# Rita-zi/WavTokenizer

Measured on AMD Instinct MI355X. Metric: audio-seconds/sec encode+decode, 24 kHz 3 s clips, higher is better.
Workload: dtype f32 (split-f16 x3 products)

## Files before the change

include/wavtokenizer_amd.h:

```cpp
#ifndef WAVTOKENIZER_AMD_H
#define WAVTOKENIZER_AMD_H

#include <stddef.h>
#include <stdint.h>

#ifdef __cplusplus
extern "C" {
#endif

typedef enum {
    WT_OK = 0,
    WT_ERR_INVALID = -1,
    WT_ERR_MISSING_TENSOR = -2,
    WT_ERR_SHAPE = -3,
    WT_ERR_HIP = -4,
    WT_ERR_NOT_INITED = -5,
    WT_ERR_RANGE = -6,
    WT_ERR_LSTM_SYNC = -7,
    WT_ERR_INDEX = -8
} wt_status;

enum wt_status_bits {
    WT_STATUS_BIT_LSTM = 1,
    WT_STATUS_BIT_RANGE = 2
// ... 37 lines not shown
    WT_PLAN_FLAG_STEP_LSTM = 4,
    WT_PLAN_FLAG_GRAPH = 8,
    WT_PLAN_FLAG_FP32_GEMM = 2,
    WT_PLAN_FLAG_RANGE_REPORT = 32,
    WT_PLAN_FLAG_MIXED_LENGTH = 64
};

enum wt_range_site {
    WT_SITE_ENCODER = 0,
    WT_SITE_BB_EMBED = 1,
    WT_SITE_RES0 = 2, WT_SITE_RES1 = 3,
    WT_SITE_ATTN = 4,
    WT_SITE_RES2 = 5, WT_SITE_RES3 = 6,
    WT_SITE_CNX0 = 7,
    WT_SITE_HEAD = 40,
    WT_SITE_SEANET_DECODER = 41
};

const char* wt_last_error(void);
const char* wt_version(void);

int  wt_model_create(const wt_arch* arch, const wt_tensor* tensors, int32_t n_tensors, int32_t device,
                     wt_model** out);
void wt_model_destroy(wt_model* m);

size_t wt_model_export_bytes(const wt_model* m);
int  wt_model_export(const wt_model* m, void* buf, size_t n);
int  wt_packed_info(const void* buf, size_t n, wt_arch* arch, int32_t* version, uint64_t* arch_hash);
int  wt_packed_verify(const void* buf, size_t n);
size_t wt_packed_bytes(const void* buf, size_t n);
int  wt_model_create_packed(const void* buf, size_t n, int32_t device, wt_model** out);
int  wt_model_hop(const wt_model* m);
int  wt_model_persistent_lstm(const wt_model* m);
int  wt_device_info(int32_t device, int32_t* compute_units, int32_t* is_gfx950, int32_t* persistent_lstm);
int64_t wt_model_weight_bytes(const wt_model* m);

int    wt_plan_create(const wt_model* m, int32_t kind, int32_t B, int64_t len, int32_t flags, wt_plan** out);
int    wt_plan_create_ex(const wt_model* m, int32_t kind, int32_t B, int64_t len, int32_t flags, uint64_t fp32_sites,
                         wt_plan** out);
void   wt_plan_destroy(wt_plan* p);
size_t wt_plan_workspace_bytes(const wt_plan* p);
int64_t wt_plan_frames(const wt_plan* p);
int    wt_plan_num_launches(const wt_plan* p);
int64_t wt_plan_graph_replays(const wt_plan* p);
int    wt_plan_find_buffer(const wt_plan* p, const char* name, size_t* offset, size_t* numel);
int    wt_plan_buffer_info(const wt_plan* p, const char* name, size_t* offset, size_t* numel, int32_t* format);
int    wt_plan_status(const wt_plan* p, int32_t* bits, int32_t clear);
int    wt_plan_range_sites(const wt_plan* p, uint64_t* sites, int32_t clear);
int    wt_plan_range_report(const wt_plan* p, int32_t index, const char** step, const char** buffer, float* amax);
int    wt_model_status(const wt_model* m, int32_t* bits, int32_t clear);
int    wt_model_split_ok(const wt_model* m);
int    wt_plan_buffer_name(const wt_plan* p, int32_t index, const char** name);

int wt_plan_num_steps(const wt_plan* p);
int wt_plan_step_name(const wt_plan* p, int32_t index, const char** name);
int wt_plan_set_timing(const wt_plan* p, const char* name_substr);
int wt_plan_read_timing(const wt_plan* p, double* total_ms, int64_t* launches, int32_t reset);

int wt_encode(const wt_plan* p, const float* wav, float* features, int64_t* codes, float* emb_out,
              void* workspace, void* stream);

int wt_encode_mixed(const wt_plan* p, const float* wav, const int32_t* lengths, float* features, int64_t* codes, float* emb_out,
                    void* workspace, void* stream);
int64_t wt_plan_min_clip_length(const wt_plan* p);
int wt_sconv_geometry(int64_t T, int32_t k, int32_t stride, int32_t dilation, int32_t out[4]);

int wt_codes_to_features(const wt_model* m, const int64_t* codes, int32_t K, int32_t B, int64_t L,
                         float* features, void* stream);

int wt_decode(const wt_plan* p, const float* features, int32_t bandwidth_id, float* wav_out,
              float* backbone_out, void* workspace, void* stream);

int wt_head(const wt_plan* p, const float* x, float* wav_out, void* workspace, void* stream);

int wt_seanet_decode(const wt_plan* p, const float* features, float* wav_out, void* workspace, void* stream);


int wt_sconv1d(const float* x, const float* w, const float* bias, float* y, int32_t B, int64_t T,
               int32_t Cin, int32_t Cout, int32_t k, int32_t stride, int32_t dilation, int32_t elu_input,
               void* stream);

int wt_linear(const float* x, const float* w, const float* bias, float* y, int64_t M, int32_t N, int32_t K,
              int32_t f16x3, void* workspace, void* stream);

int wt_conv1d_s32(const float* x, const float* w, const float* bias, float* y, int32_t B, int64_t T, int32_t Cin,
                  int32_t Cout, int32_t k, int32_t stride, int32_t zero_same, void* workspace, void* stream);

size_t wt_vq_workspace_bytes(int64_t N, int32_t D, int32_t bins);
int wt_vq_nearest(const float* x, const float* embed, int64_t N, int32_t D, int32_t bins, int64_t* codes_out,
                  void* workspace, void* stream);
int wt_vq_nearest_f32(const float* x, const float* embed, int64_t N, int32_t D, int32_t bins, int64_t* codes_out,
                      void* workspace, void* stream);

typedef struct {
    int32_t size;
    int32_t engine, epi, out, pro, b_is_act;
    int32_t M, N, K;
    int32_t T_in, T_out, Cin, taps, stride, dil, pad_left, pad_mode, Tp;
    int32_t K1, nz, tap_pair, head_kb;
    float alpha;
    int64_t a_bstride, a_rstride, a2_bstride, a2_rstride, w_rstride, c_rstride, r_rstride, zA, zW, zC;
    const float* A;
    const float* A2;
    const float* B;
    const float* bias;
    const float* R;
    const float* gamma;
    float* C;
    float* C2;
    uint32_t* status;
} wt_gemm_desc;
typedef struct {
    int32_t BM, BN, waves_m, waves_n, stages, ks, prod, staged, bias_cache, G, tiles;
} wt_launch_form;
size_t wt_gemm_probe_workspace_bytes(const wt_gemm_desc* d);
int wt_gemm_probe(const wt_gemm_desc* d, wt_launch_form* form, void* workspace, void* stream);

enum { WT_OP_GN_APPLY = 0, WT_OP_GN_STATS = 1, WT_OP_ROWNORM = 2, WT_OP_SOFTMAX = 3, WT_OP_ISTFT_OLA = 4, WT_OP_CONV_FIRST = 5,
       WT_OP_CONV_LAST = 6, WT_OP_TRANSPOSE = 7, WT_OP_CONVTR = 8, WT_OP_ROW_SUMSQ = 9, WT_OP_S32_AMAX = 10 };
enum { WT_OPK_GN_TILE = 1, WT_OPK_GN_CHUNK = 2, WT_OPK_GN_STATS = 3, WT_OPK_ROWNORM = 4, WT_OPK_DWCONV_LN = 5,
       WT_OPK_SOFTMAX_REG = 6, WT_OPK_SOFTMAX_RMW = 7, WT_OPK_ISTFT_OLA = 8, WT_OPK_CONV_FIRST = 9, WT_OPK_CONV_LAST32 = 10,
       WT_OPK_CONV_LAST = 11, WT_OPK_TRANSPOSE = 12, WT_OPK_CONVTR = 13, WT_OPK_ROW_SUMSQ = 14, WT_OPK_S32_AMAX = 15 };
typedef struct {
    int32_t size;
    int32_t op;
    int32_t B, L, C;
    int32_t groups, mode, flag, out_s32;
    int32_t ld, k, stride, Cout, n_fft, hop, Kq;
    float eps;
    int64_t n;
    const void* x;
    const void *p0, *p1, *p2, *p3, *p4, *p5;
    void *y, *y2, *y3;
    uint32_t* status;
} wt_op_desc;
typedef struct {
    int32_t kernel;
    int32_t variant;
    int32_t variant2;
    int32_t grid_x, grid_y, grid_z, block, lds;
} wt_op_form;
int wt_op_probe(const wt_op_desc* d, wt_op_form* form, void* stream);

int wt_resblock(const float* x, const float* wav, const float* e0_w, const float* e0_b, const float* w3, const float* b3,
                const float* w1, const float* b1, const float* ws, const float* bs, float* y, int32_t B, int64_t T,
                int32_t C, int32_t elu_out, int32_t out_s32, int32_t fp32_chain, void* stream);
int wt_resblock_down(const float* wav, const float* e0_w, const float* e0_b, const float* w3, const float* b3, const float* w1,
                     const float* b1, const float* ws, const float* bs, const float* wd, const float* bd, float* y_down,
                     int32_t B, int64_t T, int32_t r, void* stream);

int wt_unit_run(const wt_plan* p, const float* x, float* y, void* workspace, void* stream);

int wt_model_take_bad_codes(const wt_model* m);


typedef struct wt_resampler wt_resampler;
int     wt_resampler_create(int32_t orig_sr, int32_t new_sr, int32_t device, wt_resampler** out);
void    wt_resampler_destroy(wt_resampler* r);
int64_t wt_resampler_out_length(const wt_resampler* r, int64_t T);
int     wt_convert_audio(const wt_resampler* r, const float* wav, int32_t B, int32_t C, int64_t T, float* out, void* stream);

int wt_pcm16(const float* x, int64_t n, float limit, int32_t rescale, int16_t* out, void* workspace, void* stream);

int wt_linear_overlap_add(const float* frames, const float* weight, int32_t n_frames, int64_t rows, int64_t frame_len,
                          int64_t last_len, int64_t stride, float* out, void* stream);

#ifdef __cplusplus
}
#endif
#endif
```

wavtokenizer_amd/_capi.py:

```python
from __future__ import annotations

import ctypes
import os
from ctypes import POINTER, c_char_p, c_float, c_int32, c_int64, c_size_t, c_void_p

_HERE = os.path.dirname(os.path.abspath(__file__))
LIB_PATH = os.environ.get("WAVTOK_HIP_LIB") or os.path.join(_HERE, "libwavtok_hip.so")

EXPORTS = [
    "wt_last_error", "wt_version", "wt_model_create", "wt_model_destroy", "wt_model_export_bytes", "wt_model_export", "wt_packed_info", "wt_packed_verify", "wt_packed_bytes",
    "wt_model_create_packed", "wt_model_hop", "wt_model_weight_bytes",
    "wt_plan_create", "wt_plan_create_ex", "wt_plan_range_sites", "wt_plan_range_report", "wt_model_persistent_lstm", "wt_device_info", "wt_plan_destroy", "wt_plan_workspace_bytes", "wt_plan_frames", "wt_plan_num_launches", "wt_plan_graph_replays",
    "wt_plan_find_buffer", "wt_plan_buffer_info", "wt_plan_buffer_name", "wt_plan_status", "wt_plan_num_steps", "wt_plan_step_name",
    "wt_plan_set_timing", "wt_plan_read_timing", "wt_model_split_ok", "wt_model_status", "wt_model_take_bad_codes", "wt_encode", "wt_codes_to_features",
    "wt_decode", "wt_seanet_decode", "wt_head", "wt_unit_run", "wt_sconv1d", "wt_linear", "wt_conv1d_s32", "wt_vq_workspace_bytes",
    "wt_vq_nearest", "wt_vq_nearest_f32", "wt_resblock", "wt_resblock_down", "wt_gemm_probe_workspace_bytes", "wt_gemm_probe", "wt_op_probe",
    "wt_resampler_create", "wt_resampler_destroy", "wt_resampler_out_length", "wt_convert_audio", "wt_pcm16",
    "wt_linear_overlap_add", "wt_encode_mixed", "wt_plan_min_clip_length", "wt_sconv_geometry",
]

WT_PLAN_ENCODE, WT_PLAN_DECODE, WT_PLAN_SEANET_DECODER, WT_PLAN_HEAD, WT_PLAN_UNIT_LSTM = 0, 1, 2, 3, 4
WT_PLAN_FLAG_KEEP_STAGES = 1
WT_PLAN_FLAG_FP32_GEMM = 2
WT_PLAN_FLAG_STEP_LSTM = 4
WT_PLAN_FLAG_GRAPH = 8
WT_PLAN_FLAG_UNFUSED = 16
WT_PLAN_FLAG_RANGE_REPORT = 32
WT_PLAN_FLAG_MIXED_LENGTH = 64
WT_SITE_ENCODER, WT_SITE_BB_EMBED, WT_SITE_RES0, WT_SITE_RES1, WT_SITE_ATTN, WT_SITE_RES2, WT_SITE_RES3 = 0, 1, 2, 3, 4, 5, 6
WT_SITE_CNX0, WT_SITE_HEAD, WT_SITE_SEANET_DECODER = 7, 40, 41
WT_ERR_INVALID = -1
WT_ERR_RANGE, WT_ERR_LSTM_SYNC, WT_ERR_INDEX = -6, -7, -8
WT_STATUS_BIT_LSTM, WT_STATUS_BIT_RANGE = 1, 2
BUF_S32, BUF_ELU = 1, 2


class WtArch(ctypes.Structure):
    _fields_ = [("n_ratios", c_int32), ("ratios", c_int32 * 8), ("vq_bins", c_int32), ("num_quantizers", c_int32),
                ("input_channels", c_int32), ("dim", c_int32), ("intermediate_dim", c_int32),
                ("num_layers", c_int32), ("adanorm_num_embeddings", c_int32), ("n_fft", c_int32),
                ("hop_length", c_int32), ("padding_same", c_int32)]


class WtTensor(ctypes.Structure):
    _fields_ = [("name", c_char_p), ("data", POINTER(c_float)), ("numel", c_int64)]


class WtGemmDesc(ctypes.Structure):
    _fields_ = ([("size", c_int32), ("engine", c_int32), ("epi", c_int32), ("out", c_int32), ("pro", c_int32), ("b_is_act", c_int32),
                 ("M", c_int32), ("N", c_int32), ("K", c_int32)]
                + [(n, c_int32) for n in ("T_in", "T_out", "Cin", "taps", "stride", "dil", "pad_left", "pad_mode", "Tp",
                                         "K1", "nz", "tap_pair", "head_kb")]
                + [("alpha", c_float)]
                + [(n, c_int64) for n in ("a_bstride", "a_rstride", "a2_bstride", "a2_rstride", "w_rstride", "c_rstride",
                                         "r_rstride", "zA", "zW", "zC")]
                + [(n, c_void_p) for n in ("A", "A2", "B", "bias", "R", "gamma", "C", "C2", "status")])


class WtLaunchForm(ctypes.Structure):
    _fields_ = [(n, c_int32) for n in ("BM", "BN", "waves_m", "waves_n", "stages", "ks", "prod", "staged", "bias_cache", "G", "tiles")]


WT_OP_GN_APPLY, WT_OP_GN_STATS, WT_OP_ROWNORM, WT_OP_SOFTMAX, WT_OP_ISTFT_OLA, WT_OP_CONV_FIRST = 0, 1, 2, 3, 4, 5
WT_OP_CONV_LAST, WT_OP_TRANSPOSE, WT_OP_CONVTR, WT_OP_ROW_SUMSQ, WT_OP_S32_AMAX = 6, 7, 8, 9, 10
WT_OPK_NAMES = {1: "gn_tile", 2: "gn_chunk", 3: "gn_stats", 4: "rownorm", 5: "dwconv_ln", 6: "softmax_reg", 7: "softmax_rmw",
                8: "istft_ola", 9: "conv_first", 10: "conv_last32", 11: "conv_last", 12: "transpose", 13: "convtr",
                14: "row_sumsq", 15: "s32_amax"}


class WtOpDesc(ctypes.Structure):
    _fields_ = ([(n, c_int32) for n in ("size", "op", "B", "L", "C", "groups", "mode", "flag", "out_s32", "ld", "k", "stride",
                                        "Cout", "n_fft", "hop", "Kq")]
                + [("eps", c_float), ("n", c_int64)]
                + [(n, c_void_p) for n in ("x", "p0", "p1", "p2", "p3", "p4", "p5", "y", "y2", "y3", "status")])


class WtOpForm(ctypes.Structure):
    _fields_ = [(n, c_int32) for n in ("kernel", "variant", "variant2", "grid_x", "grid_y", "grid_z", "block", "lds")]


class WavTokError(RuntimeError):
    def __init__(self, msg, status=0):
        super().__init__(msg)
        self.status = status


def _load() -> ctypes.CDLL:
    if not os.path.exists(LIB_PATH):
        raise ImportError(
            f"{LIB_PATH} not found: build the HIP extension first (python -c 'import __graft_entry__ as g; g.build()' "
            "or make -C wavtokenizer_amd/csrc). There is no CPU fallback for the product path.")
    lib = ctypes.CDLL(LIB_PATH)
    if os.environ.get("WAVTOK_HIP_LIB"):
        class _Missing:
            def __init__(self, name):
                self.name, self.argtypes, self.restype = name, None, None

            def __call__(self, *a):
                raise WavTokError(f"{LIB_PATH} has no {self.name}")
        for sym in EXPORTS:
            try:
                getattr(lib, sym)
            except AttributeError:
                setattr(lib, sym, _Missing(sym))
    lib.wt_last_error.restype = c_char_p
    lib.wt_version.restype = c_char_p
    lib.wt_model_create.argtypes = [POINTER(WtArch), POINTER(WtTensor), c_int32, c_int32, POINTER(c_void_p)]
    lib.wt_model_destroy.argtypes = [c_void_p]
    lib.wt_model_destroy.restype = None
    lib.wt_model_export_bytes.argtypes = [c_void_p]
    lib.wt_model_export_bytes.restype = c_size_t
    lib.wt_model_export.argtypes = [c_void_p, c_void_p, c_size_t]
    lib.wt_packed_info.argtypes = [c_void_p, c_size_t, POINTER(WtArch), POINTER(c_int32), POINTER(ctypes.c_uint64)]
    lib.wt_packed_verify.argtypes = [c_void_p, c_size_t]
    lib.wt_packed_bytes.argtypes = [c_void_p, c_size_t]
    lib.wt_packed_bytes.restype = c_size_t
    lib.wt_model_create_packed.argtypes = [c_void_p, c_size_t, c_int32, POINTER(c_void_p)]
    lib.wt_model_hop.argtypes = [c_void_p]
    lib.wt_model_weight_bytes.argtypes = [c_void_p]
    lib.wt_model_weight_bytes.restype = c_int64
    lib.wt_plan_create.argtypes = [c_void_p, c_int32, c_int32, c_int64, c_int32, POINTER(c_void_p)]
    lib.wt_plan_create_ex.argtypes = [c_void_p, c_int32, c_int32, c_int64, c_int32, ctypes.c_uint64, POINTER(c_void_p)]
    lib.wt_plan_range_sites.argtypes = [c_void_p, POINTER(ctypes.c_uint64), c_int32]
    lib.wt_plan_range_report.argtypes = [c_void_p, c_int32, POINTER(c_char_p), POINTER(c_char_p), POINTER(c_float)]
    lib.wt_model_persistent_lstm.argtypes = [c_void_p]
    lib.wt_device_info.argtypes = [c_int32, POINTER(c_int32), POINTER(c_int32), POINTER(c_int32)]
    lib.wt_plan_destroy.argtypes = [c_void_p]
    lib.wt_plan_destroy.restype = None
    lib.wt_plan_workspace_bytes.argtypes = [c_void_p]
    lib.wt_plan_workspace_bytes.restype = c_size_t
    lib.wt_plan_frames.argtypes = [c_void_p]
    lib.wt_plan_frames.restype = c_int64
    lib.wt_plan_num_launches.argtypes = [c_void_p]
    lib.wt_plan_graph_replays.argtypes = [c_void_p]
    lib.wt_plan_graph_replays.restype = c_int64
    lib.wt_plan_find_buffer.argtypes = [c_void_p, c_char_p, POINTER(c_size_t), POINTER(c_size_t)]
    lib.wt_plan_buffer_info.argtypes = [c_void_p, c_char_p, POINTER(c_size_t), POINTER(c_size_t), POINTER(c_int32)]
    lib.wt_plan_status.argtypes = [c_void_p, POINTER(c_int32), c_int32]
    lib.wt_model_split_ok.argtypes = [c_void_p]
    lib.wt_model_status.argtypes = [c_void_p, POINTER(c_int32), c_int32]
    lib.wt_model_take_bad_codes.argtypes = [c_void_p]
    lib.wt_unit_run.argtypes = [c_void_p, c_void_p, c_void_p, c_void_p, c_void_p]
    lib.wt_plan_buffer_name.argtypes = [c_void_p, c_int32, POINTER(c_char_p)]
    lib.wt_plan_num_steps.argtypes = [c_void_p]
    lib.wt_plan_step_name.argtypes = [c_void_p, c_int32, POINTER(c_char_p)]
    lib.wt_plan_set_timing.argtypes = [c_void_p, c_char_p]
    lib.wt_plan_read_timing.argtypes = [c_void_p, POINTER(ctypes.c_double), POINTER(c_int64), c_int32]
    lib.wt_encode.argtypes = [c_void_p, c_void_p, c_void_p, c_void_p, c_void_p, c_void_p, c_void_p]
    lib.wt_encode_mixed.argtypes = [c_void_p, c_void_p, c_void_p, c_void_p, c_void_p, c_void_p, c_void_p, c_void_p]
    lib.wt_plan_min_clip_length.argtypes = [c_void_p]
    lib.wt_plan_min_clip_length.restype = c_int64
    lib.wt_sconv_geometry.argtypes = [c_int64, c_int32, c_int32, c_int32, POINTER(c_int32)]
    lib.wt_codes_to_features.argtypes = [c_void_p, c_void_p, c_int32, c_int32, c_int64, c_void_p, c_void_p]
    lib.wt_decode.argtypes = [c_void_p, c_void_p, c_int32, c_void_p, c_void_p, c_void_p, c_void_p]
    lib.wt_seanet_decode.argtypes = [c_void_p, c_void_p, c_void_p, c_void_p, c_void_p]
    lib.wt_head.argtypes = [c_void_p, c_void_p, c_void_p, c_void_p, c_void_p]
    lib.wt_sconv1d.argtypes = [c_void_p, c_void_p, c_void_p, c_void_p, c_int32, c_int64, c_int32, c_int32, c_int32,
                               c_int32, c_int32, c_int32, c_void_p]
    lib.wt_linear.argtypes = [c_void_p, c_void_p, c_void_p, c_void_p, c_int64, c_int32, c_int32, c_int32, c_void_p, c_void_p]
    lib.wt_conv1d_s32.argtypes = [c_void_p, c_void_p, c_void_p, c_void_p, c_int32, c_int64, c_int32, c_int32, c_int32,
                                  c_int32, c_int32, c_void_p, c_void_p]
    lib.wt_vq_workspace_bytes.argtypes = [c_int64, c_int32, c_int32]
    lib.wt_vq_workspace_bytes.restype = c_size_t
    lib.wt_vq_nearest.argtypes = [c_void_p, c_void_p, c_int64, c_int32, c_int32, c_void_p, c_void_p, c_void_p]
    lib.wt_vq_nearest_f32.argtypes = [c_void_p, c_void_p, c_int64, c_int32, c_int32, c_void_p, c_void_p, c_void_p]
    lib.wt_resblock.argtypes = [c_void_p] * 11 + [c_int32, c_int64, c_int32, c_int32, c_int32, c_int32, c_void_p]
    lib.wt_resblock_down.argtypes = [c_void_p] * 12 + [c_int32, c_int64, c_int32, c_void_p]
    lib.wt_gemm_probe_workspace_bytes.argtypes = [POINTER(WtGemmDesc)]
    lib.wt_gemm_probe_workspace_bytes.restype = c_size_t
    lib.wt_gemm_probe.argtypes = [POINTER(WtGemmDesc), POINTER(WtLaunchForm), c_void_p, c_void_p]
    lib.wt_op_probe.argtypes = [POINTER(WtOpDesc), POINTER(WtOpForm), c_void_p]
    lib.wt_resampler_create.argtypes = [c_int32, c_int32, c_int32, POINTER(c_void_p)]
    lib.wt_resampler_destroy.argtypes = [c_void_p]
    lib.wt_resampler_destroy.restype = None
    lib.wt_resampler_out_length.argtypes = [c_void_p, c_int64]
    lib.wt_resampler_out_length.restype = c_int64
    lib.wt_convert_audio.argtypes = [c_void_p, c_void_p, c_int32, c_int32, c_int64, c_void_p, c_void_p]
    lib.wt_pcm16.argtypes = [c_void_p, c_int64, ctypes.c_float, c_int32, c_void_p, c_void_p, c_void_p]
    lib.wt_linear_overlap_add.argtypes = [c_void_p, c_void_p, c_int32, c_int64, c_int64, c_int64, c_int64, c_void_p, c_void_p]
    return lib


lib = _load()


def check(rc: int, what: str = "") -> None:
    if rc != 0:
        msg = lib.wt_last_error()
        raise WavTokError(f"{what} failed (status {rc}): {msg.decode() if msg else ''}", rc)
```

wavtokenizer_amd/csrc/capi.cpp:

```cpp
#include "model.h"

namespace wt {
static thread_local std::string g_err;
void set_error(const std::string& msg) { g_err = msg; }
thread_local LaunchCtx g_launch;
int device_cus() {
    static std::atomic<int> cache[64];
    int d = 0;
    (void)hipGetDevice(&d);
    d &= 63;
    int v = cache[d].load(std::memory_order_relaxed);
    if (v <= 0) {
        if (hipDeviceGetAttribute(&v, hipDeviceAttributeMultiprocessorCount, d) != hipSuccess || v <= 0) v = 256;
        cache[d].store(v, std::memory_order_relaxed);
    }
    return v;
}
}

using namespace wt;

static int alloc_host_words(wt_model* M, const char* who) {
    void* hp = nullptr;
    void* dp = nullptr;
// ... 547 lines not shown
    return run_plan(p, c);
}

int wt_decode(const wt_plan* p, const float* features, int32_t bandwidth_id, float* wav_out, float* backbone_out,
              void* workspace, void* stream) {
    if (!p || p->kind != WT_PLAN_DECODE) { set_error("wt_decode: not a decode plan"); return WT_ERR_INVALID; }
    if (!features || !wav_out || !workspace) { set_error("wt_decode: null buffer"); return WT_ERR_INVALID; }
    if (bandwidth_id < 0 || bandwidth_id >= p->model->arch.adanorm_num_embeddings) {
        set_error("wt_decode: bandwidth_id out of range"); return WT_ERR_INVALID;
    }
    RunCtx c{static_cast<char*>(workspace), static_cast<hipStream_t>(stream), features, wav_out, nullptr, backbone_out, bandwidth_id};
    return run_plan(p, c);
}

int wt_head(const wt_plan* p, const float* x, float* wav_out, void* workspace, void* stream) {
    if (!p || p->kind != WT_PLAN_HEAD) { set_error("wt_head: wrong plan kind"); return WT_ERR_INVALID; }
    if (!x || !wav_out || !workspace) { set_error("wt_head: null buffer"); return WT_ERR_INVALID; }
    RunCtx c{static_cast<char*>(workspace), static_cast<hipStream_t>(stream), x, wav_out, nullptr, nullptr, 0};
    return run_plan(p, c);
}

int wt_seanet_decode(const wt_plan* p, const float* features, float* wav_out, void* workspace, void* stream) {
    if (!p || p->kind != WT_PLAN_SEANET_DECODER) { set_error("wt_seanet_decode: wrong plan kind"); return WT_ERR_INVALID; }
    if (!features || !wav_out || !workspace) { set_error("wt_seanet_decode: null buffer"); return WT_ERR_INVALID; }
    RunCtx c{static_cast<char*>(workspace), static_cast<hipStream_t>(stream), features, wav_out, nullptr, nullptr, 0};
    return run_plan(p, c);
}

int wt_unit_run(const wt_plan* p, const float* x, float* y, void* workspace, void* stream) {
    if (!p || p->kind != WT_PLAN_UNIT_LSTM) { set_error("wt_unit_run: wrong plan kind"); return WT_ERR_INVALID; }
    if (!x || !y || !workspace) { set_error("wt_unit_run: null buffer"); return WT_ERR_INVALID; }
    RunCtx c{static_cast<char*>(workspace), static_cast<hipStream_t>(stream), x, y, nullptr, nullptr, 0};
    return run_plan(p, c);
}

int wt_codes_to_features(const wt_model* m, const int64_t* codes, int32_t K, int32_t B, int64_t L, float* features,
                         void* stream) {
    if (!m || !codes || !features) { set_error("wt_codes_to_features: null argument"); return WT_ERR_INVALID; }
    if (K < 1 || K > m->arch.num_quantizers) { set_error("wt_codes_to_features: K exceeds the number of codebooks"); return WT_ERR_INVALID; }
    DeviceGuard dg(m->device);
    if (!dg.ok) { set_error("hipSetDevice failed"); return WT_ERR_HIP; }
    return launch_codes_to_features(codes, m->embed.w, K, m->arch.vq_bins, B, L, 512, features, static_cast<hipStream_t>(stream),
                                    m->bad_codes_dev);
}

int wt_sconv1d(const float* x, const float* w, const float* bias, float* y, int32_t B, int64_t T, int32_t Cin,
               int32_t Cout, int32_t k, int32_t stride, int32_t dilation, int32_t elu_input, void* stream) {
    ConvW cw; cw.w = const_cast<float*>(w); cw.b = const_cast<float*>(bias); cw.cout = Cout; cw.cin = Cin; cw.k = k;
    GemmArgs a = sconv_args(cw, B, T, stride, dilation);
    a.A = x; a.C = y;
    return launch_gemm(a, elu_input ? PRO_ELU : PRO_NONE, EPI_BIAS, static_cast<hipStream_t>(stream));
}

static int split_pair(const float* w, long nw, const float* x, long nx, char* ws_w, char* ws_x, char* tail, GemmArgs& a,
                      hipStream_t s) {
    unsigned* bits = reinterpret_cast<unsigned*>(tail);
    float* sc = reinterpret_cast<float*>(tail + 16);
    if (int rc = launch_pow2_scales(w, nw, x, nx, bits, sc, s)) return rc;
    if (int rc = launch_split_s32(w, ws_w, nw, s, sc)) return rc;
    if (int rc = launch_split_s32(x, ws_x, nx, s, sc + 1)) return rc;
    a.W_hi = ws_w;
    a.A = reinterpret_cast<const float*>(ws_x);
    a.acc_scale_dev = sc + 2;
    return 0;
}

int wt_linear(const float* x, const float* w, const float* bias, float* y, int64_t M, int32_t N, int32_t K,
              int32_t f16x3, void* workspace, void* stream) {
    if (!x || !w || !y) { set_error("wt_linear: null argument"); return WT_ERR_INVALID; }
    hipStream_t s = static_cast<hipStream_t>(stream);
    GemmArgs a = linear_args(w, bias, M, N, K);
    a.A = x; a.C = y;
    if (!f16x3) return launch_gemm(a, PRO_NONE, EPI_BIAS, s);
    if (!workspace) { set_error("wt_linear: the f16x3 modes need a workspace"); return WT_ERR_INVALID; }
    char* hi = static_cast<char*>(workspace);
    if (f16x3 == 1) { set_error("wt_linear: mode 1 (the in-loop split kernel of round 1) was removed; use 2, 3 or 4"); return WT_ERR_INVALID; }
    char* xs = hi + (size_t)N * K * 4;
    if (int rc = split_pair(w, (long)N * K, x, (long)M * K, hi, xs, xs + (size_t)M * K * 4, a, s)) return rc;
    a.dbg_stamps = reinterpret_cast<unsigned long long*>(xs + (size_t)M * K * 4 + 256);
    if (f16x3 == 4) return launch_gemm16s(a, EPI_BIAS_GELU, OUT_S32, s);
    return launch_gemm16s(a, EPI_BIAS, f16x3 == 3 ? 1 : 0, s);
}

int wt_conv1d_s32(const float* x, const float* w, const float* bias, float* y, int32_t B, int64_t T, int32_t Cin,
                  int32_t Cout, int32_t k, int32_t stride, int32_t zero_same, void* workspace, void* stream) {
    if (!x || !w || !y || !workspace) { set_error("wt_conv1d_s32: null argument"); return WT_ERR_INVALID; }
    hipStream_t s = static_cast<hipStream_t>(stream);
    ConvW cw; cw.w = const_cast<float*>(w); cw.b = const_cast<float*>(bias); cw.cout = Cout; cw.cin = Cin; cw.k = k;
    GemmArgs a = zero_same ? zconv_args(cw, B, (int)T) : sconv_args(cw, B, T, stride, 1);
    char* ws = static_cast<char*>(workspace);
    char* xs = ws + (size_t)Cout * k * Cin * 4;
    if (int rc = split_pair(w, (long)Cout * k * Cin, x, (long)B * T * Cin, ws, xs, xs + (size_t)B * T * Cin * 4, a, s)) return rc;
    a.C = y;
    return launch_gemm16s(a, EPI_BIAS, 0, s);
}

static size_t al256(size_t b) { return (b + 255) / 256 * 256; }

struct ProbeLayout { long nA = 0, nA2 = 0, nB = 0; size_t oA2 = 0, oB = 0, oScale = 0, total = 0; };
static ProbeLayout probe_layout(const wt_gemm_desc& d) {
    ProbeLayout L;
    const long clips = d.M / d.T_out;
    const long a_cols = d.A2 ? d.K1 : d.Cin;
    L.nA = (d.nz - 1) * d.zA + (clips - 1) * d.a_bstride + (long)(d.T_in - 1) * d.a_rstride + a_cols;
    if (d.A2) L.nA2 = (clips - 1) * d.a2_bstride + (long)(d.T_in - 1) * d.a2_rstride + (d.K - d.K1);
    L.nB = (d.nz - 1) * d.zW + (long)(d.N - 1) * d.w_rstride + d.K;
    L.oA2 = al256((size_t)L.nA * 4);
    L.oB = L.oA2 + al256((size_t)L.nA2 * 4);
    L.oScale = L.oB + al256((size_t)L.nB * 4);
    L.total = L.oScale + 256;
    return L;
}
static int probe_args(const wt_gemm_desc* d, char* ws, GemmArgs& a) {
    if (!d || d->size != (int32_t)sizeof(wt_gemm_desc)) { set_error("wt_gemm_probe: descriptor missing or of another size"); return WT_ERR_INVALID; }
    if (d->engine != 0 && d->engine != 1) { set_error("wt_gemm_probe: engine is 0 (gemm16s) or 1 (gemm)"); return WT_ERR_INVALID; }
    if (!d->A || !d->B || !d->C) { set_error("wt_gemm_probe: A, B and C are required"); return WT_ERR_INVALID; }
    if (d->epi == EPI_ARGMAX) { set_error("wt_gemm_probe: the argmax epilogue is reached through wt_vq_nearest"); return WT_ERR_INVALID; }
    if (d->M <= 0 || d->N <= 0 || d->K <= 0 || d->T_out <= 0 || d->T_in <= 0 || d->M % d->T_out || d->nz < 1 || d->taps < 1 ||
        d->stride < 1 || d->dil < 1 || d->pad_left < 0 || (d->pad_mode != PAD_ZERO && d->pad_mode != PAD_REFLECT) ||
        d->a_bstride < 0 || d->a_rstride < 0 || d->a2_bstride < 0 || d->a2_rstride < 0 || d->w_rstride < d->K ||
        d->c_rstride < d->N || d->r_rstride < 0 || d->zA < 0 || d->zW < 0 || d->zC < 0 || (d->nz > 1 && d->zC <= 0)) {
        set_error("wt_gemm_probe: bad extents or strides"); return WT_ERR_INVALID;
    }
    if (d->engine == 1 && (d->out != OUT_F32 || d->A2 || d->tap_pair)) {
        set_error("wt_gemm_probe: gemm.hip writes fp32 and has no second K source or tap pairing"); return WT_ERR_INVALID;
    }
    if (d->engine == 0 && d->pro != PRO_NONE) { set_error("wt_gemm_probe: gemm16s has no operand prologue"); return WT_ERR_INVALID; }
    if (d->tap_pair && (d->taps != 2 * d->stride || d->dil != 1)) { set_error("wt_gemm_probe: tap pairing needs k = 2 * stride, dilation 1"); return WT_ERR_INVALID; }
    if (d->engine == 0 && (!ws || (reinterpret_cast<uintptr_t>(ws) & 255))) { set_error("wt_gemm_probe: gemm16s needs a 256-byte aligned workspace"); return WT_ERR_INVALID; }
    a = GemmArgs{};
    a.a_bstride = d->a_bstride; a.a_rstride = d->a_rstride; a.T_in = d->T_in; a.T_out = d->T_out; a.Cin = d->Cin; a.taps = d->taps;
    a.stride = d->stride; a.dil = d->dil; a.pad_left = d->pad_left; a.pad_mode = d->pad_mode; a.Tp = d->Tp;
    a.a2_bstride = d->a2_bstride; a.a2_rstride = d->a2_rstride; a.K1 = d->K1;
    a.w_rstride = d->w_rstride; a.bias = d->bias; a.M = d->M; a.N = d->N; a.K = d->K;
    a.C = d->C; a.c_rstride = d->c_rstride; a.C2 = d->C2; a.R = d->R; a.r_rstride = d->r_rstride; a.gamma = d->gamma;
    a.alpha = d->alpha; a.nz = d->nz; a.zA = d->zA; a.zW = d->zW; a.zC = d->zC; a.head_kb = d->head_kb; a.tap_pair = d->tap_pair ? 1 : 0;
    if (d->engine == 1) {
        a.A = d->A; a.W = d->B;
        return check_gemm(a, d->pro, d->epi) ? WT_ERR_INVALID : WT_OK;
    }
    const ProbeLayout L = probe_layout(*d);
    a.A = reinterpret_cast<const float*>(ws);
    a.A2 = d->A2 ? reinterpret_cast<const float*>(ws + L.oA2) : nullptr;
    a.W = d->B; a.W_hi = ws + L.oB;
    a.status = reinterpret_cast<unsigned*>(d->status);
    return check_gemm16s(a, d->epi, d->out) ? WT_ERR_INVALID : WT_OK;
}

size_t wt_gemm_probe_workspace_bytes(const wt_gemm_desc* d) {
    if (!d || d->size != (int32_t)sizeof(wt_gemm_desc) || d->engine != 0 || d->M <= 0 || d->T_out <= 0 || d->nz < 1) return 0;
    return probe_layout(*d).total;
}

int wt_gemm_probe(const wt_gemm_desc* d, wt_launch_form* form, void* workspace, void* stream) {
    char* ws = static_cast<char*>(workspace);
    GemmArgs a;
    if (int rc = probe_args(d, ws, a)) return rc;
    hipStream_t s = static_cast<hipStream_t>(stream);
    LaunchForm lf;
    a.form = &lf;
    if (d->engine == 1) {
        if (int rc = launch_gemm(a, d->pro, d->epi, s)) return rc;
    } else {
        const ProbeLayout L = probe_layout(*d);
        float* scale_dev = reinterpret_cast<float*>(ws + L.oScale);
        float scale = 1.f;
        if (!d->b_is_act) {
            std::vector<float> h((size_t)L.nB);
            WT_HIP_CHECK(hipMemcpyAsync(h.data(), d->B, (size_t)L.nB * 4, hipMemcpyDeviceToHost, s));
            WT_HIP_CHECK(hipStreamSynchronize(s));
            float amax = 0.f;
            for (long z = 0; z < d->nz; ++z)
                for (long n = 0; n < d->N; ++n)
                    for (long k = 0; k < d->K; ++k) {
                        const float v = std::fabs(h[(size_t)(z * d->zW + n * d->w_rstride + k)]);
                        if (!(v <= 3.0e38f)) { set_error("wt_gemm_probe: a non-finite weight has no S32 copy"); return WT_ERR_INVALID; }
                        amax = std::max(amax, v);
                    }
            scale = s32_weight_scale(amax);
            uint32_t bits;
            memcpy(&bits, &scale, 4);
            if (int rc = launch_fill_u32(scale_dev, bits, 16, s)) return rc;
            a.acc_scale = 1.f / scale;
        }
        if (int rc = launch_split_s32(d->B, ws + L.oB, L.nB, s, scale != 1.f ? scale_dev : nullptr)) return rc;
        if (int rc = launch_split_s32(d->A, ws, L.nA, s)) return rc;
        if (d->A2) if (int rc = launch_split_s32(d->A2, ws + L.oA2, L.nA2, s)) return rc;
        if (int rc = launch_gemm16s(a, d->epi, d->out, s)) return rc;
    }
    if (form) *form = wt_launch_form{lf.BM, lf.BN, lf.waves_m, lf.waves_n, lf.stages, lf.ks, lf.prod, lf.staged, lf.bias_cache, lf.G, lf.tiles};
    return WT_OK;
}

static int op_probe_check(const wt_op_desc* d) {
    auto bad = [](const char* m) { set_error(std::string("wt_op_probe: ") + m); return (int)WT_ERR_INVALID; };
    if (!d || d->size != (int32_t)sizeof(wt_op_desc)) return bad("descriptor missing or of another size");
    if (d->op < WT_OP_GN_APPLY || d->op > WT_OP_S32_AMAX) return bad("unknown op");
    auto al16 = [](const void* p) { return !(reinterpret_cast<uintptr_t>(p) & 15); };
    const void* ptrs[] = {d->p0, d->p1, d->p2, d->p3, d->p4, d->p5, d->y, d->y2, d->y3};
    for (const void* p : ptrs) if (!al16(p)) return bad("arrays must be 16-byte aligned");
    if (!d->x || (reinterpret_cast<uintptr_t>(d->x) & (d->op == WT_OP_SOFTMAX ? 3 : 15))) return bad("x missing or misaligned");
    if (reinterpret_cast<uintptr_t>(d->status) & 3) return bad("status misaligned");
    const bool shaped = d->op != WT_OP_SOFTMAX && d->op != WT_OP_ROW_SUMSQ && d->op != WT_OP_S32_AMAX;
    if (shaped && (d->B <= 0 || d->L <= 0)) return bad("extents must be positive");
    if (shaped && d->op != WT_OP_CONV_FIRST && d->op != WT_OP_ISTFT_OLA && (d->C <= 0 || (long)d->L * d->C >= (long)INT_MAX)) return bad("extents must be positive (and L * C < 2^31)");
    switch (d->op) {
    case WT_OP_GN_APPLY: case WT_OP_GN_STATS:
        if (!d->p0 || !d->p1 || !d->y2 || !d->y3 || (d->op == WT_OP_GN_APPLY && !d->y)) return bad("null argument");
        if (d->groups <= 0 || d->C % d->groups || d->C / d->groups > 256 || d->B > 65535) return bad("GroupNorm needs C % groups == 0, at most 256 channels per group, B <= 65535");
        break;
    case WT_OP_ROWNORM:
        if (!d->y || !d->p4 || !d->p5) return bad("null argument");
        if (d->mode < RN_DWCONV || d->mode > RN_AFFINE_IN) return bad("rownorm mode is 0, 1 or 2");
        if (d->mode == RN_DWCONV && (!d->p0 || !d->p1)) return bad("null argument");
        if (d->mode == RN_AFFINE_IN && (!d->p2 || !d->p3)) return bad("null argument");
        break;
    case WT_OP_SOFTMAX:
        if (d->n <= 0 || d->n > INT_MAX || d->L <= 0 || d->ld < d->L) return bad("softmax needs rows > 0 and 0 < L <= ld");
        break;
    case WT_OP_ISTFT_OLA:
        if (!d->p0 || !d->p1 || !d->y) return bad("null argument");
        if (d->n_fft <= 0 || d->hop <= 0 || d->n_fft % 4 || d->n_fft % d->hop || (d->n_fft - d->hop) % 2 || d->Kq < d->n_fft / 4 + 1)
            return bad("the ISTFT tail needs n_fft % 4 == 0, n_fft % hop == 0 and Kq > n_fft / 4");
        break;
    case WT_OP_CONV_FIRST:
        if (!d->p0 || !d->p1 || !d->y) return bad("null argument");
        if (d->k <= 0 || d->Cout <= 0 || d->Cout % 4) return bad("conv_first needs k > 0 and Cout % 4 == 0");
        break;
    case WT_OP_CONV_LAST:
        if (!d->p0 || !d->p1 || !d->y) return bad("null argument");
        if (d->k <= 0) return bad("conv_last needs k > 0");
        break;
    case WT_OP_TRANSPOSE:
        if (!d->y) return bad("null argument");
        if (d->B > 65535 || (d->L + 31) / 32 > 65535) return bad("transpose: too many tiles for one launch");
        break;
    case WT_OP_CONVTR:
        if (!d->p0 || !d->p1 || !d->y) return bad("null argument");
        if (d->stride <= 0 || d->k < d->stride || d->Cout <= 0 || d->Cout % 4) return bad("convtr needs k >= stride > 0 and Cout % 4 == 0");
        break;
    case WT_OP_ROW_SUMSQ:
        if (!d->y) return bad("null argument");
        if (d->n <= 0 || d->C <= 0 || d->C % 4) return bad("row_sumsq needs rows > 0 and C % 4 == 0");
        break;
    case WT_OP_S32_AMAX:
        if (!d->y) return bad("null argument");
        if (d->n <= 0 || d->n % 32) return bad("s32_amax needs whole S32 groups of 32 values");
        break;
    }
    return WT_OK;
}

int wt_op_probe(const wt_op_desc* d, wt_op_form* form, void* stream) {
    if (int rc = op_probe_check(d)) return rc;
    hipStream_t s = static_cast<hipStream_t>(stream);
    auto F = [](const void* p) { return static_cast<const float*>(p); };
    auto W = [](void* p) { return static_cast<float*>(p); };
    OpForm lf;
    const LaunchCtx saved = g_launch;
    g_launch.status = reinterpret_cast<unsigned*>(d->status);
    g_launch.form = &lf;
    int rc = 0;
    switch (d->op) {
    case WT_OP_GN_APPLY:
        rc = launch_gn_apply(F(d->x), F(d->p0), F(d->p1), W(d->y2), W(d->y3), W(d->y), d->flag ? 1 : 0, d->B, d->L, d->C, d->groups, d->eps, s,
                             d->out_s32 ? 1 : 0, const_cast<float*>(F(d->p2)));
        break;
    case WT_OP_GN_STATS:
        rc = launch_gn_stats(F(d->x), F(d->p0), F(d->p1), W(d->y2), W(d->y3), d->B, d->L, d->C, d->groups, d->eps, s, const_cast<float*>(F(d->p2)));
        break;
    case WT_OP_ROWNORM:
        rc = launch_rownorm(d->mode, F(d->x), W(d->y), d->B, d->L, d->C, F(d->p0), F(d->p1), F(d->p2), F(d->p3), F(d->p4), F(d->p5), d->eps, s,
                            d->out_s32 ? 1 : 0);
        break;
    case WT_OP_SOFTMAX:
        rc = launch_softmax(const_cast<float*>(F(d->x)), (int)d->n, d->L, d->ld, s, W(d->y));
        break;
    case WT_OP_ISTFT_OLA:
        rc = launch_istft_ola(F(d->x), F(d->p0), F(d->p1), W(d->y), d->B, d->L, d->n_fft, d->hop, d->Kq, d->flag ? 1 : 0, s);
        break;
    case WT_OP_CONV_FIRST:
        rc = launch_conv_first(F(d->x), F(d->p0), F(d->p1), W(d->y), d->B, d->L, d->k, d->Cout, s);
        break;
    case WT_OP_CONV_LAST:
        rc = launch_conv_last(F(d->x), F(d->p0), F(d->p1), W(d->y), d->B, d->L, d->C, d->k, d->flag ? 1 : 0, s);
        break;
    case WT_OP_TRANSPOSE:
        rc = launch_transpose(F(d->x), W(d->y), d->B, d->L, d->C, s, d->out_s32 ? 1 : 0);
        break;
    case WT_OP_CONVTR:
        rc = launch_convtr(F(d->x), F(d->p0), F(d->p1), W(d->y), d->B, d->L, d->C, d->Cout, d->k, d->stride, d->flag ? 1 : 0, s);
        break;
    case WT_OP_ROW_SUMSQ:
        rc = launch_row_sumsq(F(d->x), W(d->y), d->n, d->C, s);
        break;
    case WT_OP_S32_AMAX:
        rc = launch_s32_amax(d->x, d->n, static_cast<unsigned*>(d->y), s);
        break;
    }
    g_launch = saved;
    if (rc) return rc;
    if (form) *form = wt_op_form{lf.kernel, lf.variant, lf.variant2, (int32_t)lf.grid[0], (int32_t)lf.grid[1], (int32_t)lf.grid[2], (int32_t)lf.block, (int32_t)lf.lds};
    return WT_OK;
}

size_t wt_vq_workspace_bytes(int64_t N, int32_t D, int32_t bins) {
    const size_t np = std::max(gemm_vq_parts(bins), gemm16s_vq_parts(bins));
    return al256((size_t)N * D * 4) + al256((size_t)bins * D * 4) + al256((size_t)N * sizeof(float)) +
           2 * al256((size_t)N * np * sizeof(float)) + al256((size_t)bins * sizeof(float)) + 512;
}

static int vq_nearest(const float* x, const float* embed, int64_t N, int32_t D, int32_t bins, int64_t* codes_out,
                      void* workspace, void* stream, bool s32) {
    if (!x || !embed || !codes_out || !workspace) { set_error("wt_vq_nearest: null argument"); return WT_ERR_INVALID; }
    if (s32 && (D % 32)) { set_error("wt_vq_nearest: the split-f16 kernel needs D % 32 == 0"); return WT_ERR_INVALID; }
    hipStream_t s = static_cast<hipStream_t>(stream);
    const int np = s32 ? gemm16s_vq_parts(bins) : gemm_vq_parts(bins);
    char* ws = static_cast<char*>(workspace);
    char* xs = ws; ws += al256((size_t)N * D * 4);
    char* es = ws; ws += al256((size_t)bins * D * 4);
    float* xx = reinterpret_cast<float*>(ws); ws += al256((size_t)N * sizeof(float));
    float* pv = reinterpret_cast<float*>(ws); ws += al256((size_t)N * np * sizeof(float));
    int* pi = reinterpret_cast<int*>(ws); ws += al256((size_t)N * np * sizeof(float));
    float* ee = reinterpret_cast<float*>(ws); ws += al256((size_t)bins * sizeof(float));
    if (int rc = launch_row_sumsq(x, xx, N, D, s)) return rc;
    if (int rc = launch_row_sumsq(embed, ee, bins, D, s)) return rc;
    GemmArgs a = linear_args(embed, nullptr, N, bins, D);
    a.A = x; a.vq_xx = xx; a.vq_ee = ee; a.vq_pval = pv; a.vq_pidx = pi; a.vq_nparts = np;
    if (s32) {
        if (int rc = split_pair(embed, (long)bins * D, x, (long)N * D, es, xs, ws, a, s)) return rc;
        if (int rc = launch_gemm16s(a, EPI_ARGMAX, OUT_F32, s)) return rc;
    } else {
        if (int rc = launch_gemm(a, PRO_NONE, EPI_ARGMAX, s)) return rc;
    }
    for (int64_t r0 = 0; r0 < N; r0 += 8192) {
        const int n = (int)std::min<int64_t>(8192, N - r0);
        if (int rc = launch_vq_finalize(pv + r0 * np, pi + r0 * np, np, embed, codes_out + r0, nullptr, 1, n, D, bins, s)) return rc;
    }
    return WT_OK;
}
int wt_vq_nearest(const float* x, const float* embed, int64_t N, int32_t D, int32_t bins, int64_t* codes_out,
                  void* workspace, void* stream) {
    return vq_nearest(x, embed, N, D, bins, codes_out, workspace, stream, true);
}
int wt_vq_nearest_f32(const float* x, const float* embed, int64_t N, int32_t D, int32_t bins, int64_t* codes_out,
                      void* workspace, void* stream) {
    return vq_nearest(x, embed, N, D, bins, codes_out, workspace, stream, false);
}

// ... 33 lines not shown
```

wavtokenizer_amd/csrc/common.h:

```cpp
#pragma once
#include <hip/hip_runtime.h>
#include <stdint.h>
#include <stdio.h>
#include <stdlib.h>
#include <mutex>
#include <string>

namespace wt {

void set_error(const std::string& msg);

#define WT_HIP_CHECK(expr)                                                                      \
    do {                                                                                        \
        hipError_t _e = (expr);                                                                 \
        if (_e != hipSuccess) {                                                                 \
            ::wt::set_error(std::string(#expr) + ": " + hipGetErrorString(_e));                 \
            return -4;                                                                          \
        }                                                                                       \
    } while (0)

struct PerDeviceOnce {
    std::mutex mu;
    bool seen[64] = {};
    template <class F> int run(F&& f) {
// ... 122 lines not shown
    EPI_BIAS_ROW = 8,
    EPI_BIAS_RES_ELU = 9,
    EPI_BIAS_ELU = 10
};
enum Out16s : int {
    OUT_F32 = 0,
    OUT_S32 = 1,
    OUT_S32_DUAL_ELU = 2,
    OUT_F32_AND_S32 = 3
};
enum PadMode : int { PAD_ZERO = 0, PAD_REFLECT = 1 };

struct LaunchForm {
    int BM = 0, BN = 0, waves_m = 0, waves_n = 0, stages = 0;
    int ks = 1, prod = 0;
    int staged = 0, bias_cache = 0;
    int G = 0, tiles = 0;
};

struct GemmArgs {
    const float* A = nullptr;
    long a_bstride = 0;
    long a_rstride = 0;
    int T_in = 0, T_out = 0;
    int Cin = 0, taps = 1, stride = 1, dil = 1, pad_left = 0, pad_mode = PAD_ZERO;
    int Tp = 0;
    const float* A2 = nullptr;
    long a2_bstride = 0, a2_rstride = 0;
    int K1 = 0;
    const float* W = nullptr;
    long w_rstride = 0;
    const void* W_hi = nullptr;
    const float* bias = nullptr;
    int M = 0, N = 0, K = 0;
    float* C = nullptr;
    long c_rstride = 0;
    float* C2 = nullptr;
    const float* R = nullptr;
    long r_rstride = 0;
    const float* gamma = nullptr;
    float alpha = 1.f;
    int nz = 1;
    long zA = 0, zW = 0, zC = 0;
    int head_kb = 0;
    const float* vq_xx = nullptr;
    const float* vq_ee = nullptr;
    float* vq_pval = nullptr;
    int*   vq_pidx = nullptr;
    int vq_nparts = 0;
    int group_m = 8;
    int group_n = 0;
    int tap_pair = 0;
    unsigned long long* stamp_start = nullptr;
    unsigned long long* stamp_end = nullptr;
    int stage_epi = 0;
    int stage_off = 0;
    int pc_off = 0;
    float acc_scale = 1.f;
    const float* acc_scale_dev = nullptr;
    unsigned* status = nullptr;
    unsigned long long* dbg_stamps = nullptr;
    LaunchForm* form = nullptr;
};

int gemm_vq_parts(int N);
int check_gemm(const GemmArgs& a, int pro, int epi);
int check_gemm16s(const GemmArgs& a, int epi, int out, const int* mix_geom = nullptr);
int launch_gemm(const GemmArgs& a, int pro, int epi, hipStream_t s);
int launch_gemm16s(const GemmArgs& a, int epi, int out, hipStream_t s, const int* mix_geom = nullptr);
int gemm16s_vq_parts(int N);
int launch_split_s32(const float* x, void* out, long n, hipStream_t s, const float* scale_dev = nullptr);
int launch_unsplit_s32(const void* s32, float* out, long n, float inv_scale, hipStream_t s);
int launch_pow2_scales(const float* a, long na, const float* b, long nb, unsigned* bits2, float* out3, hipStream_t s);

int launch_conv_first(const float* wav, const float* w , const float* bias, float* y, int B, long T,
                      int k, int Cout, hipStream_t s);
int launch_conv_last(const float* x , const float* w , const float* bias, float* y ,
                     int B, long T, int Cin, int k, int elu_in, hipStream_t s);
int launch_transpose(const float* in, float* out, int B, int R, int C, hipStream_t s, int out_s32 = 0);
size_t gn_part_floats(int B, int L, int groups);
int launch_gn_stats(const float* x, const float* gamma, const float* beta, float* scale, float* shift, int B, int L,
                    int C, int groups, float eps, hipStream_t s, float* part = nullptr);
int launch_gn_apply(const float* x, const float* gamma, const float* beta, float* scale, float* shift, float* y,
                    int swish, int B, int L, int C, int groups, float eps, hipStream_t s, int out_s32 = 0, float* part = nullptr);
enum RowNormMode : int { RN_DWCONV = 0, RN_PLAIN = 1, RN_AFFINE_IN = 2 };
int launch_rownorm(int mode, const float* x, float* y, int B, int L, int C, const float* dw_w ,
                   const float* dw_b, const float* in_scale, const float* in_shift, const float* out_scale,
                   const float* out_shift, float eps, hipStream_t s, int out_s32 = 0);
int launch_istft_ola(const float* parts, const float* win, const float* wsq, float* out, int B, int L, int n_fft, int hop,
                     int Kq, int center, hipStream_t s);
int launch_softmax(float* S, int rows, int L, int ld, hipStream_t s, float* P_s32 = nullptr);
int launch_row_sumsq(const float* x, float* out, long rows, int D, hipStream_t s);
int launch_vq_finalize(const float* pval, const int* pidx, int nparts, const float* embed, int64_t* codes,
                       float* feat_ncl, int B, int L, int D, int bins, hipStream_t s);
int launch_codes_to_features(const int64_t* codes, const float* embed, int K, int bins, int B, long L, int D,
                             float* feat_ncl, hipStream_t s, unsigned* bad = nullptr);
int launch_fill_u32(void* p, unsigned value, size_t n_bytes, hipStream_t s);
int launch_plan_guard(const unsigned* status, int nwords, int site0, unsigned* host_status, unsigned* model_status, int64_t* codes,
                      long n_codes, float* f0, long n0, float* f1, long n1, float* f2, long n2, hipStream_t s);
int launch_s32_amax(const void* s32, long numel, unsigned* out_bits, hipStream_t s);
struct LstmArgs {
    const float* xg0;
    const float* W0;
    const float* W1;
    const float* b1;
    float* h0;
    float* h1;
    float* c0;
    float* c1;
    const float* x;
    float* y;
    int B, L, H;
    int elu_out;
    int out_s32;
    int f16x3;
    unsigned* status = nullptr;
};
int launch_lstm_step(const LstmArgs& a, int s, hipStream_t stream);
struct LstmPersistArgs {
    const float* xg0;
    const void* Wp;
    const float* b1;
    const float* x;
    float* y;
    void* hx;
    unsigned* ctl;
    unsigned* status = nullptr;
    int dbg_spin_shift = 0;
    int B, L, H, Bx;
    int elu_out, out_s32;
    int data_flag;
};
size_t lstm_persist_hx_bytes();
size_t lstm_persist_ctl_bytes();
int launch_lstm_persist(const LstmPersistArgs& a, hipStream_t stream);
struct ResblockArgs {
    const float* x;
    const float* wav;
    const float* e0_w;
    const float* e0_b;
    const float* W3;
    const float* b3;
    const float* W1;
    const float* b1;
    const float* Ws;
    const float* bs;
    float* y;
    int B, T, C;
    long x_bstride;
    int elu_out;
    int out_s32;
    int dbg;
    unsigned* status;
    const float* Wd;
    const float* bd;
    float* y_down;
    int R;
};
struct ResblockMix {
    const int* T = nullptr;
    const int* Tread = nullptr;
};
bool resblock_fusable(int C);
int launch_resblock(const ResblockArgs& a, hipStream_t s);
int launch_resblock16(const ResblockArgs& a, hipStream_t s, const ResblockMix* mix = nullptr);
bool resblock16_down_fusable(int C, long T, int r, int k);
int launch_resblock16_down(const ResblockArgs& a, hipStream_t s, const ResblockMix* mix = nullptr);
// ... 9 lines not shown
```

wavtokenizer_amd/csrc/model.h:

```cpp
#pragma once
#include "../../include/wavtokenizer_amd.h"
#include "common.h"

#include <algorithm>
#include <atomic>
#include <climits>
#include <cmath>
#include <cstring>
#include <functional>
#include <map>
#include <memory>
#include <mutex>
#include <string>
#include <vector>

namespace wt {

struct S32Copy {
    const void* p = nullptr;
    float acc_scale = 1.f;
    bool tap_pair = false;
};
struct ConvW {
    float* w = nullptr;
    float* b = nullptr;
    int cout = 0, cin = 0, k = 0;
    S32Copy s32;
};
struct GemmW {
    float* w = nullptr;
    int rows = 0, cols = 0;
    S32Copy s32;
};
struct LstmW {
    GemmW Wih0;
    float* b0 = nullptr;
    float* W0 = nullptr;
    float* W1 = nullptr;
    float* b1 = nullptr;
    float* W0h = nullptr;
    float* W1h = nullptr;
    float* Wp = nullptr;
};
struct ResStage {
    ConvW c3, c1, sc, down;
    ConvW cat;
    int C = 0, r = 0;
};
struct PosRes {
    float *n1w, *n1b, *n2w, *n2b;
    ConvW c1, c2;
};
struct CnxBlock {
    float *dw_w, *dw_b, *ada_s, *ada_h, *b1, *b2, *gamma;
    GemmW W1, W2;
};
struct SeaDecStage {
    float* tr_w = nullptr;
    GemmW tr_wp;
    float* tr_b = nullptr;
    int cin = 0, cout = 0, k = 0, r = 0;
    ConvW c3, c1, sc;
    ConvW cat;
};

}

struct wt_model {
    wt_arch arch{};
    int device = 0;
    int hop = 1;
    int H = 512;
    std::vector<int> enc_ratios;
    std::vector<void*> allocs;
    std::vector<size_t> alloc_bytes;
    int64_t weight_bytes = 0;
    float *e0_w = nullptr, *e0_b = nullptr;
    int e0_k = 7, e0_c = 32;
    std::vector<wt::ResStage> stages;
    wt::LstmW enc_lstm;
    wt::ConvW enc_final;
    wt::GemmW embed;
    float* ee = nullptr;
    wt::ConvW bb_embed;
    wt::PosRes res[4];
    float *at_nw, *at_nb, *at_bqk, *at_bv, *at_bp;
    wt::GemmW at_Wqk, at_Wv, at_Wp;
    float *gn5w, *gn5b, *ada_s, *ada_h;
    std::vector<wt::CnxBlock> cnx;
    float *fln_w, *fln_b;
    wt::GemmW head_W, istft_W;
    float *head_b = nullptr, *wsq = nullptr, *win = nullptr;
    int Kb = 0, Kq = 0, bins_f = 0, R = 0;
    bool has_seadec = false;
    wt::ConvW sd_first;
    wt::LstmW sd_lstm;
    std::vector<wt::SeaDecStage> sd_stages;
    float *sd_last_w = nullptr, *sd_last_b = nullptr;
    bool s32_ok = true;
    bool sd_s32_ok = true;
    float w_amax = 0.f;
    struct LazyF32 { const float* w; const void* s32; int64_t n; float scale; };
    std::vector<LazyF32> lazy_f32;
    mutable std::atomic<bool> f32_stale{false};
    mutable std::mutex f32_mu;
    unsigned* bad_codes_host = nullptr;
    unsigned* bad_codes_dev = nullptr;
    unsigned* status_host = nullptr;
    unsigned* status_dev = nullptr;
    mutable std::atomic<bool> persist_ok{true};
};

namespace wt {

struct TensorMap {
    std::map<std::string, std::pair<const float*, int64_t>> m;
    std::string missing;
    const float* get(const std::string& k, int64_t numel) {
        auto it = m.find(k);
        if (it == m.end()) { if (missing.empty()) missing = k; return nullptr; }
        if (it->second.second != numel) {
            if (missing.empty()) missing = k + " (numel " + std::to_string(it->second.second) + ", expected " + std::to_string(numel) + ")";
            return nullptr;
        }
        return it->second.first;
    }
    bool has(const std::string& k) const { return m.count(k) != 0; }
};

struct RunCtx {
    char* ws;
    hipStream_t stream;
    const float* in_f;
    float* out_f;
    int64_t* codes;
    float* aux;
    int bw_id;
    const int* lengths = nullptr;
};
enum Site : int {
    SITE_ENC = 0,
    SITE_BB_EMBED = 1,
    SITE_RES0 = 2, SITE_RES1 = 3, SITE_ATTN = 4, SITE_RES2 = 5, SITE_RES3 = 6,
    SITE_CNX0 = 7,
    SITE_HEAD = 40,
    SITE_SEADEC = 41,
    SITE_COUNT = 64
};
constexpr int CTL_SITE0 = 16;
constexpr int CTL_WORDS = CTL_SITE0 + SITE_COUNT + 48;

enum BufFmt : int { BUF_F32 = 0, BUF_S32 = 1, BUF_ELU = 2 };
struct BufSpec {
    std::string name;
    size_t bytes = 0, numel = 0, off = 0;
    int first = INT_MAX, last = -1;
    int fmt = BUF_F32;
};

struct DeviceGuard {
    int prev = -1;
    bool ok = true;
    explicit DeviceGuard(int dev) {
        if (hipGetDevice(&prev) != hipSuccess) prev = -1;
        if (prev != dev) ok = hipSetDevice(dev) == hipSuccess; else prev = -1;
    }
    ~DeviceGuard() { if (prev >= 0) (void)hipSetDevice(prev); }
};

}
// ... 33 lines not shown
    struct GraphKey {
        const void *ws = nullptr, *in = nullptr, *out = nullptr, *codes = nullptr, *aux = nullptr, *lengths = nullptr;
        int bw = -1;
        bool operator==(const GraphKey& o) const {
            return ws == o.ws && in == o.in && out == o.out && codes == o.codes && aux == o.aux && lengths == o.lengths && bw == o.bw;
        }
    };
    mutable GraphKey graph_key, last_key;
    mutable bool graph_failed = false;
    mutable hipGraphExec_t graph_exec = nullptr;
    mutable hipStream_t cap_stream = nullptr;
    mutable long graph_replays = 0;

    wt_plan() = default;
    wt_plan(const wt_plan&) = delete;
    ~wt_plan() {
        if (status_host) (void)hipHostFree(status_host);
        if (range_dev) (void)hipFree(range_dev);
        if (stamps) (void)hipFree(stamps);
        if (graph_exec) (void)hipGraphExecDestroy(graph_exec);
        if (cap_stream) (void)hipStreamDestroy(cap_stream);
        for (auto& ev : ev_pending) { (void)hipEventDestroy(ev.first); (void)hipEventDestroy(ev.second); }
        for (auto& ev : ev_free) { (void)hipEventDestroy(ev.first); (void)hipEventDestroy(ev.second); }
    }

    int buf(const std::string& name, size_t numel, int fmt = wt::BUF_F32) {
        wt::BufSpec b;
        b.name = name; b.numel = numel; b.bytes = (numel * sizeof(float) + 255) / 256 * 256; b.fmt = fmt;
        bufs.push_back(b);
        return (int)bufs.size() - 1;
    }
    void step(std::initializer_list<int> used, std::function<int(const wt::RunCtx&)> fn, int launches = 1,
              const std::string& name = "") {
        const int s = (int)steps.size();
        std::string nm = name;
        for (int id : used) {
            if (id < 0) continue;
            bufs[id].first = std::min(bufs[id].first, s);
            bufs[id].last = std::max(bufs[id].last, s);
            if (name.empty()) nm = bufs[id].name;
        }
        if (flags & WT_PLAN_FLAG_RANGE_REPORT)
            for (int id : used)
                if (id >= 0 && (bufs[id].fmt & wt::BUF_S32)) range_entries.push_back({s, id});
        steps.push_back(std::move(fn));
        step_names.push_back(nm);
        step_sites.push_back(cur_site);
        n_launches += launches;
    }
    float* ptr(const wt::RunCtx& c, int id) const { return reinterpret_cast<float*>(c.ws + bufs[id].off); }
    void layout() {
        const bool keep = flags & WT_PLAN_FLAG_KEEP_STAGES;
        std::vector<int> order(bufs.size());
        for (size_t i = 0; i < order.size(); ++i) order[i] = (int)i;
        std::stable_sort(order.begin(), order.end(), [&](int x, int y) { return bufs[x].first < bufs[y].first; });
        std::vector<int> placed;
        ws_bytes = 0;
        for (int id : order) {
            wt::BufSpec& b = bufs[id];
            if (b.last < 0) { b.off = 0; continue; }
            if (keep) b.last = INT_MAX;
            size_t off = 0;
            bool moved = true;
            while (moved) {
                moved = false;
                for (int pid : placed) {
                    const wt::BufSpec& q = bufs[pid];
                    const bool live = !(q.last < b.first || b.last < q.first);
                    const bool overlap = off < q.off + q.bytes && q.off < off + b.bytes;
                    if (live && overlap) { off = q.off + q.bytes; moved = true; }
                }
            }
            b.off = off;
            placed.push_back(id);
            ws_bytes = std::max(ws_bytes, off + b.bytes);
        }
        ws_bytes = std::max<size_t>(ws_bytes, 256);
    }
};

namespace wt {

int build_model(wt_model* M, TensorMap& tm);
int build_splits(wt_model* M);
float s32_weight_scale(float amax);
size_t model_export_bytes(const wt_model* M);
int model_export(const wt_model* M, void* buf, size_t n);
int model_import(wt_model* M, const void* buf, size_t n);
int packed_info(const void* buf, size_t n, wt_arch* arch, int32_t* version, uint64_t* arch_hash);
int ensure_f32_weights(const wt_model* M);
size_t packed_bytes(const void* buf, size_t n);
int packed_verify(const void* buf, size_t n);
GemmArgs sconv_args(const ConvW& w, int B, long T, int stride, int dil);
GemmArgs zconv_args(const ConvW& w, int B, int L);
GemmArgs linear_args(const float* W, const float* bias, long M, int N, int K);
GemmArgs linear_args(const GemmW& W, const float* bias, long M, int N, int K);
int build_encode(wt_plan* P);
int build_decode(wt_plan* P);
int build_head(wt_plan* P);
int build_seanet_decoder(wt_plan* P);
int build_unit_lstm(wt_plan* P);
void plan_begin(wt_plan* P);
void plan_end(wt_plan* P);
inline long wave_samples(const wt_model* M, long L) {
    return M->arch.padding_same ? L * (long)M->arch.hop_length : (L - 1) * (long)M->arch.hop_length;
}

}
```

wavtokenizer_amd/csrc/ops.hip:

```cpp
#include "common.h"
#include <stdlib.h>

namespace wt {

typedef float f32x4 __attribute__((ext_vector_type(4)));

static inline void note_form(int kernel, int variant, int variant2, dim3 grid, unsigned block, size_t lds = 0) {
    if (OpForm* f = g_launch.form) *f = OpForm{kernel, variant, variant2, {grid.x, grid.y, grid.z}, block, (unsigned)lds};
}

__device__ __forceinline__ float wave_sum(float v) {
#pragma unroll
    for (int off = 32; off >= 1; off >>= 1) v += __shfl_xor(v, off, 64);
    return v;
}
typedef _Float16 f16x4s __attribute__((ext_vector_type(4)));
__device__ __forceinline__ void store_s32_1(float* row_base, int e, float v, float& amax) {
    amax = amax1(amax, v);
    _Float16* p = reinterpret_cast<_Float16*>(row_base) + ((e >> 5) * 64 + (e & 31));
    const _Float16 h = (_Float16)v;
    p[0] = h;
    p[32] = (_Float16)((v - (float)h) * 2048.f);
}
__device__ __forceinline__ void store_s32_4(float* row_base, int e, const f32x4 v, float& amax) {
// ... 176 lines not shown
    range_report(status, amax);
}

int launch_transpose(const float* in, float* out, int B, int R, int C, hipStream_t s, int out_s32) {
    if (out_s32 && (R % 32)) { set_error("transpose: an S32 output needs rows in multiples of 32 elements"); return -1; }
    dim3 grid((C + 31) / 32, (R + 31) / 32, B);
    note_form(OPK_TRANSPOSE, 0, 0, grid, 256);
    hipLaunchKernelGGL(transpose_kernel, grid, dim3(256), 0, s, in, out, R, C, out_s32, g_launch.status);
    WT_HIP_CHECK(hipGetLastError());
    return 0;
}

template <int APPLY>
__global__ __launch_bounds__(256) void gn_stats_kernel(const float* __restrict__ x, const float* __restrict__ gamma,
                                                       const float* __restrict__ beta, float* __restrict__ scale,
                                                       float* __restrict__ shift, float* __restrict__ y, int L, int C,
                                                       int cg, float eps, int s32, unsigned* status) {
    __shared__ float red[4];
    float amax = 0.f;
    __shared__ float s_mean, s_rstd;
    const int g = blockIdx.x, b = blockIdx.y;
    const float* xb = x + (long)b * L * C + g * cg;
    const int n = L * cg;
    const int lane = threadIdx.x & 63, wv = threadIdx.x >> 6;
    float sum = 0.f;
    for (int i = threadIdx.x; i < n; i += 256) {
        const int t = i / cg, j = i - t * cg;
        sum += xb[(long)t * C + j];
    }
    sum = wave_sum(sum);
    if (lane == 0) red[wv] = sum;
    __syncthreads();
    if (threadIdx.x == 0) s_mean = (red[0] + red[1] + red[2] + red[3]) / (float)n;
    __syncthreads();
    const float mean = s_mean;
    float sq = 0.f;
    for (int i = threadIdx.x; i < n; i += 256) {
        const int t = i / cg, j = i - t * cg;
        const float d = xb[(long)t * C + j] - mean;
        sq += d * d;
    }
    sq = wave_sum(sq);
    __syncthreads();
    if (lane == 0) red[wv] = sq;
    __syncthreads();
    if (threadIdx.x == 0) s_rstd = 1.f / sqrtf((red[0] + red[1] + red[2] + red[3]) / (float)n + eps);
    __syncthreads();
    if (threadIdx.x < cg) {
        const int c = g * cg + threadIdx.x;
        const float sc = s_rstd * gamma[c];
        scale[(long)b * C + c] = sc;
        shift[(long)b * C + c] = beta[c] - mean * sc;
    }
    if (APPLY) {
        float* yb = y + (long)b * L * C + g * cg;
        const float rstd = s_rstd;
        for (int i = threadIdx.x; i < n; i += 256) {
            const int t = i / cg, j = i - t * cg;
            const float sc = rstd * gamma[g * cg + j];
            float v = xb[(long)t * C + j] * sc + (beta[g * cg + j] - mean * sc);
            if (APPLY == 2) v = v / (1.f + expf(-v));
            if (s32) store_s32_1(y + ((long)b * L + t) * C, g * cg + j, v, amax);
            else yb[(long)t * C + j] = v;
        }
        range_report(status, amax);
    }
}

static int launch_gn_chunked(const float*, const float*, const float*, float*, float*, float*, int, int, int, int, int, int, float,
                             hipStream_t, int, float*);
static int gn_slab_groups(int C, int groups);
int launch_gn_stats(const float* x, const float* gamma, const float* beta, float* scale, float* shift, int B, int L,
                    int C, int groups, float eps, hipStream_t s, float* part) {
    const int GBs = gn_slab_groups(C, groups), cgs = C / groups;
    if (part && L > 256 && GBs && (cgs % 4 == 0) && (C % 4 == 0) && GBs <= 8)
        return launch_gn_chunked(x, gamma, beta, scale, shift, nullptr, 0, B, L, C, groups, GBs, eps, s, 0, part);
    note_form(OPK_GN_STATS, 0, 0, dim3(groups, B), 256);
    hipLaunchKernelGGL(gn_stats_kernel<0>, dim3(groups, B), dim3(256), 0, s, x, gamma, beta, scale, shift,
                       (float*)nullptr, L, C, C / groups, eps, 0, (unsigned*)nullptr);
    WT_HIP_CHECK(hipGetLastError());
    return 0;
}

template <int SWISH>
__global__ __launch_bounds__(512) void gn_tile_kernel(const float* __restrict__ x, const float* __restrict__ gamma,
                                                      const float* __restrict__ beta, float* __restrict__ scale,
                                                      float* __restrict__ shift, float* __restrict__ y, int L, int C,
                                                      int cg, int GB, float eps, int s32, unsigned* status) {
    extern __shared__ __attribute__((aligned(16))) float tile[];
    float amax = 0.f;
    __shared__ float s_sc[128], s_sh[128], s_red[8];
    const int NT = blockDim.x;
    const int W = GB * cg, W4 = W / 4;
    const int c0 = blockIdx.x * W, b = blockIdx.y;
    const float* xb = x + (long)b * L * C + c0;
    const int dt = NT / W4, dq = NT - dt * W4;
    {
        int t = threadIdx.x / W4, q = threadIdx.x - t * W4;
        for (; t < L; t += dt, q += dq) {
            if (q >= W4) { q -= W4; ++t; if (t >= L) break; }
            *reinterpret_cast<f32x4*>(tile + t * W + q * 4) = *reinterpret_cast<const f32x4*>(xb + (long)t * C + q * 4);
        }
    }
    __syncthreads();
    const int lane = threadIdx.x & 63, wv = threadIdx.x >> 6, nw = NT >> 6;
    if (nw == 2 * GB) {
        const int gl = wv >> 1, part = wv & 1;
        const int r0 = part ? L / 2 : 0, r1 = part ? L : L / 2;
        const int n = L * cg;
        const float* col = tile + gl * cg;
        const int cg4 = cg >> 2, rp = 64 / cg4, lr = lane / cg4, lq = lane - lr * cg4;
        float sum = 0.f;
        if (lr < rp)
            for (int t = r0 + lr; t < r1; t += rp) {
                const f32x4 v = *reinterpret_cast<const f32x4*>(col + t * W + lq * 4);
                sum += (v.x + v.y) + (v.z + v.w);
            }
        sum = wave_sum(sum);
        if (lane == 0) s_red[wv] = sum;
        __syncthreads();
        const float mean = (s_red[2 * gl] + s_red[2 * gl + 1]) / (float)n;
        __syncthreads();
        float sq = 0.f;
        if (lr < rp)
            for (int t = r0 + lr; t < r1; t += rp) {
                const f32x4 v = *reinterpret_cast<const f32x4*>(col + t * W + lq * 4);
                const float dx = v.x - mean, dy = v.y - mean, dz = v.z - mean, dw = v.w - mean;
                sq += (dx * dx + dy * dy) + (dz * dz + dw * dw);
            }
        sq = wave_sum(sq);
        if (lane == 0) s_red[wv] = sq;
        __syncthreads();
        const float rstd = 1.f / sqrtf((s_red[2 * gl] + s_red[2 * gl + 1]) / (float)n + eps);
        if (part == 0 && lane < cg) {
            const int c = c0 + gl * cg + lane;
            const float sc = rstd * gamma[c], sh = beta[c] - mean * sc;
            s_sc[gl * cg + lane] = sc; s_sh[gl * cg + lane] = sh;
            scale[(long)b * C + c] = sc; shift[(long)b * C + c] = sh;
        }
    } else
    for (int gl = wv; gl < GB; gl += nw) {
        const int n = L * cg;
        const float* col = tile + gl * cg;
        const int cg4 = cg >> 2, rp = 64 / cg4, lr = lane / cg4, lq = lane - lr * cg4;
        float sum = 0.f;
        if (lr < rp)
            for (int t = lr; t < L; t += rp) {
                const f32x4 v = *reinterpret_cast<const f32x4*>(col + t * W + lq * 4);
                sum += (v.x + v.y) + (v.z + v.w);
            }
        const float mean = wave_sum(sum) / (float)n;
        float sq = 0.f;
        if (lr < rp)
            for (int t = lr; t < L; t += rp) {
                const f32x4 v = *reinterpret_cast<const f32x4*>(col + t * W + lq * 4);
                const float dx = v.x - mean, dy = v.y - mean, dz = v.z - mean, dw = v.w - mean;
                sq += (dx * dx + dy * dy) + (dz * dz + dw * dw);
            }
        const float rstd = 1.f / sqrtf(wave_sum(sq) / (float)n + eps);
        if (lane < cg) {
            const int c = c0 + gl * cg + lane;
            const float sc = rstd * gamma[c], sh = beta[c] - mean * sc;
            s_sc[gl * cg + lane] = sc; s_sh[gl * cg + lane] = sh;
            scale[(long)b * C + c] = sc; shift[(long)b * C + c] = sh;
        }
    }
    __syncthreads();
    float* yb = y + (long)b * L * C;
    {
        int t = threadIdx.x / W4, q = threadIdx.x - t * W4;
        for (; t < L; t += dt, q += dq) {
            if (q >= W4) { q -= W4; ++t; if (t >= L) break; }
            const f32x4 v = *reinterpret_cast<const f32x4*>(tile + t * W + q * 4);
            const f32x4 sc = *reinterpret_cast<const f32x4*>(s_sc + q * 4), sh = *reinterpret_cast<const f32x4*>(s_sh + q * 4);
            f32x4 o = v * sc + sh;
            if (SWISH) {
                o.x *= __builtin_amdgcn_rcpf(1.f + __expf(-o.x)); o.y *= __builtin_amdgcn_rcpf(1.f + __expf(-o.y));
                o.z *= __builtin_amdgcn_rcpf(1.f + __expf(-o.z)); o.w *= __builtin_amdgcn_rcpf(1.f + __expf(-o.w));
            }
            if (s32) store_s32_4(yb + (long)t * C, c0 + q * 4, o, amax);
            else *reinterpret_cast<f32x4*>(yb + (long)t * C + c0 + q * 4) = o;
        }
    }
    range_report(status, amax);
}

static constexpr int GN_CH = 128;
__global__ __launch_bounds__(256) void gn_chunk_stats_kernel(const float* __restrict__ x, float* __restrict__ part, int L,
                                                             int C, int cg, int GB, int groups, int nch) {
    extern __shared__ __attribute__((aligned(16))) float tile[];
    const int W = GB * cg, W4 = W / 4;
    const int c0 = blockIdx.x * W, k = blockIdx.y, b = blockIdx.z;
    const int t0 = k * GN_CH, rows = L - t0 < GN_CH ? L - t0 : GN_CH;
    const float* xb = x + ((long)b * L + t0) * C + c0;
    for (int e = threadIdx.x; e < rows * W4; e += 256) {
        const int t = e / W4, q = e - t * W4;
        *reinterpret_cast<f32x4*>(tile + t * W + q * 4) = *reinterpret_cast<const f32x4*>(xb + (long)t * C + q * 4);
    }
    __syncthreads();
    const int lane = threadIdx.x & 63, wv = threadIdx.x >> 6;
    for (int gl = wv; gl < GB; gl += 4) {
        const float* col = tile + gl * cg;
        const int cg4 = cg >> 2, rp = 64 / cg4, lr = lane / cg4, lq = lane - lr * cg4;
        float sum = 0.f;
        if (lr < rp)
            for (int t = lr; t < rows; t += rp) {
                const f32x4 v = *reinterpret_cast<const f32x4*>(col + t * W + lq * 4);
                sum += (v.x + v.y) + (v.z + v.w);
            }
        const float mean = wave_sum(sum) / (float)(rows * cg);
        float sq = 0.f;
        if (lr < rp)
            for (int t = lr; t < rows; t += rp) {
                const f32x4 v = *reinterpret_cast<const f32x4*>(col + t * W + lq * 4);
                const float dx = v.x - mean, dy = v.y - mean, dz = v.z - mean, dw = v.w - mean;
                sq += (dx * dx + dy * dy) + (dz * dz + dw * dw);
            }
        sq = wave_sum(sq);
        if (lane == 0) {
            float* o = part + (((long)b * groups + blockIdx.x * GB + gl) * nch + k) * 2;
            o[0] = mean; o[1] = sq;
        }
    }
}

template <int APPLY>
__global__ __launch_bounds__(256) void gn_chunk_apply_kernel(const float* __restrict__ x, const float* __restrict__ part,
                                                             const float* __restrict__ gamma, const float* __restrict__ beta,
                                                             float* __restrict__ scale, float* __restrict__ shift,
                                                             float* __restrict__ y, int L, int C, int cg, int GB, int groups,
                                                             int nch, float eps, int s32, unsigned* status) {
    __shared__ float s_mean[8], s_rstd[8], s_sc[128], s_sh[128];
    float amax = 0.f;
    const int W = GB * cg, W4 = W / 4;
    const int c0 = blockIdx.x * W, k = blockIdx.y, b = blockIdx.z;
    if (threadIdx.x < GB) {
        const float* pp = part + ((long)b * groups + blockIdx.x * GB + threadIdx.x) * nch * 2;
        float n = 0.f, mean = 0.f, m2 = 0.f;
        for (int q = 0; q < nch; ++q) {
            const int rows = L - q * GN_CH < GN_CH ? L - q * GN_CH : GN_CH;
            const float nq = (float)(rows * cg), d = pp[2 * q] - mean, tot = n + nq;
            mean += d * (nq / tot);
            m2 += pp[2 * q + 1] + d * d * (n * nq / tot);
            n = tot;
        }
        s_mean[threadIdx.x] = mean;
        s_rstd[threadIdx.x] = 1.f / sqrtf(m2 / n + eps);
    }
    __syncthreads();
    if (threadIdx.x < W) {
        const int c = c0 + threadIdx.x, gl = threadIdx.x / cg;
        const float sc = s_rstd[gl] * gamma[c], sh = beta[c] - s_mean[gl] * sc;
        s_sc[threadIdx.x] = sc; s_sh[threadIdx.x] = sh;
        if (k == 0) { scale[(long)b * C + c] = sc; shift[(long)b * C + c] = sh; }
    }
    if (APPLY == 0) return;
    __syncthreads();
    const int t0 = k * GN_CH, rows = L - t0 < GN_CH ? L - t0 : GN_CH;
    const float* xb = x + ((long)b * L + t0) * C + c0;
    float* yb = y + ((long)b * L + t0) * C;
    for (int e = threadIdx.x; e < rows * W4; e += 256) {
        const int t = e / W4, q = e - t * W4;
        const f32x4 v = *reinterpret_cast<const f32x4*>(xb + (long)t * C + q * 4);
        const f32x4 sc = *reinterpret_cast<const f32x4*>(s_sc + q * 4), sh = *reinterpret_cast<const f32x4*>(s_sh + q * 4);
        f32x4 o = v * sc + sh;
        if (APPLY == 2) {
            o.x *= __builtin_amdgcn_rcpf(1.f + __expf(-o.x)); o.y *= __builtin_amdgcn_rcpf(1.f + __expf(-o.y));
            o.z *= __builtin_amdgcn_rcpf(1.f + __expf(-o.z)); o.w *= __builtin_amdgcn_rcpf(1.f + __expf(-o.w));
        }
        if (s32) store_s32_4(yb + (long)t * C, c0 + q * 4, o, amax);
        else *reinterpret_cast<f32x4*>(yb + (long)t * C + c0 + q * 4) = o;
    }
    range_report(status, amax);
}

size_t gn_part_floats(int B, int L, int groups) { return (size_t)B * groups * ((L + GN_CH - 1) / GN_CH) * 2; }

static int launch_gn_chunked(const float* x, const float* gamma, const float* beta, float* scale, float* shift, float* y,
                             int mode, int B, int L, int C, int groups, int GB, float eps, hipStream_t s, int out_s32,
                             float* part) {
    const int cg = C / groups, nch = (L + GN_CH - 1) / GN_CH;
    const size_t smem = (size_t)GN_CH * GB * cg * sizeof(float);
    static PerDeviceOnce attr_once;
    if (int rc = attr_once.run([&]() -> int { WT_HIP_CHECK(hipFuncSetAttribute(reinterpret_cast<const void*>(gn_chunk_stats_kernel), hipFuncAttributeMaxDynamicSharedMemorySize, 64 * 1024)); return 0; })) return rc;
    hipLaunchKernelGGL(gn_chunk_stats_kernel, dim3(groups / GB, nch, B), dim3(256), smem, s, x, part, L, C, cg, GB, groups, nch);
    const dim3 grid(groups / GB, mode ? nch : 1, B);
    note_form(OPK_GN_CHUNK, mode, 0, grid, 256, smem);
    if (mode == 0) hipLaunchKernelGGL(gn_chunk_apply_kernel<0>, grid, dim3(256), 0, s, x, part, gamma, beta, scale, shift, y, L, C, cg, GB, groups, nch, eps, out_s32, g_launch.status);
    else if (mode == 1) hipLaunchKernelGGL(gn_chunk_apply_kernel<1>, grid, dim3(256), 0, s, x, part, gamma, beta, scale, shift, y, L, C, cg, GB, groups, nch, eps, out_s32, g_launch.status);
    else hipLaunchKernelGGL(gn_chunk_apply_kernel<2>, grid, dim3(256), 0, s, x, part, gamma, beta, scale, shift, y, L, C, cg, GB, groups, nch, eps, out_s32, g_launch.status);
    WT_HIP_CHECK(hipGetLastError());
    return 0;
}
static int gn_slab_groups(int C, int groups) {
    const int cg = C / groups;
    for (int g = 1; g <= groups; ++g)
        if (groups % g == 0 && (g * cg) % 32 == 0 && g * cg <= 128) return g;
    return 0;
}

int launch_gn_apply(const float* x, const float* gamma, const float* beta, float* scale, float* shift, float* y,
                    int swish, int B, int L, int C, int groups, float eps, hipStream_t s, int out_s32, float* part) {
    if (out_s32 && (C % 32)) { set_error("gn_apply: an S32 output needs C % 32 == 0"); return -1; }
    const int cg = C / groups;
    int GB = 0;
    for (int g = 1; g <= groups; ++g)
        if (groups % g == 0 && (g * cg) % 32 == 0 && g * cg <= 128) { GB = g; break; }
    if (GB && (cg % 4 == 0) && (size_t)L * GB * cg * 4 <= 96 * 1024 && (C % 4 == 0)) {
        const size_t smem = (size_t)L * GB * cg * sizeof(float);
        static PerDeviceOnce attr_once;
        if (int rc = attr_once.run([&]() -> int {
            WT_HIP_CHECK(hipFuncSetAttribute(reinterpret_cast<const void*>(gn_tile_kernel<0>), hipFuncAttributeMaxDynamicSharedMemorySize, 96 * 1024));
            WT_HIP_CHECK(hipFuncSetAttribute(reinterpret_cast<const void*>(gn_tile_kernel<1>), hipFuncAttributeMaxDynamicSharedMemorySize, 96 * 1024));
        return 0;
    })) return rc;
        dim3 grid(groups / GB, B);
        const int nt = GB == 4 ? 512 : 256;
        note_form(OPK_GN_TILE, swish ? 1 : 0, (nt >> 6) == 2 * GB ? 2 : 1, grid, nt, smem);
        if (swish) hipLaunchKernelGGL(gn_tile_kernel<1>, grid, dim3(nt), smem, s, x, gamma, beta, scale, shift, y, L, C, cg, GB, eps, out_s32, g_launch.status);
        else hipLaunchKernelGGL(gn_tile_kernel<0>, grid, dim3(nt), smem, s, x, gamma, beta, scale, shift, y, L, C, cg, GB, eps, out_s32, g_launch.status);
        WT_HIP_CHECK(hipGetLastError());
        return 0;
    }
    if (part && GB && (cg % 4 == 0) && (C % 4 == 0) && GB * cg <= 128 && GB <= 8)
        return launch_gn_chunked(x, gamma, beta, scale, shift, y, swish ? 2 : 1, B, L, C, groups, GB, eps, s, out_s32, part);
    note_form(OPK_GN_STATS, swish ? 2 : 1, 0, dim3(groups, B), 256);
    if (swish)
        hipLaunchKernelGGL(gn_stats_kernel<2>, dim3(groups, B), dim3(256), 0, s, x, gamma, beta, scale, shift, y, L, C,
                           C / groups, eps, out_s32, g_launch.status);
    else
        hipLaunchKernelGGL(gn_stats_kernel<1>, dim3(groups, B), dim3(256), 0, s, x, gamma, beta, scale, shift, y, L, C,
                           C / groups, eps, out_s32, g_launch.status);
    WT_HIP_CHECK(hipGetLastError());
    return 0;
}

template <int NV, int MODE>
__global__ __launch_bounds__(256) void rownorm_kernel(const float* __restrict__ x, float* __restrict__ y, long M, int L,
                                                      const float* __restrict__ dw_w, const float* __restrict__ dw_b,
                                                      const float* __restrict__ in_scale,
                                                      const float* __restrict__ in_shift,
                                                      const float* __restrict__ out_scale,
                                                      const float* __restrict__ out_shift, float eps, int s32, unsigned* status) {
    constexpr int C = NV * 256;
    const int lane = threadIdx.x & 63;
    float amax = 0.f;
    const long m = (long)blockIdx.x * 4 + (threadIdx.x >> 6);
    if (m >= M) return;
    const long b = m / L;
    const int t = (int)(m - b * L);
    f32x4 v[NV];
#pragma unroll
    for (int i = 0; i < NV; ++i) {
        const int c = (i * 64 + lane) * 4;
        if (MODE == RN_DWCONV) {
            f32x4 acc = *reinterpret_cast<const f32x4*>(dw_b + c);
#pragma unroll
            for (int j = 0; j < 7; ++j) {
                const int tt = t + j - 3;
                if (tt >= 0 && tt < L) {
                    const f32x4 xv = *reinterpret_cast<const f32x4*>(x + (b * L + tt) * C + c);
                    const f32x4 wv = *reinterpret_cast<const f32x4*>(dw_w + j * C + c);
                    acc += xv * wv;
                }
            }
            v[i] = acc;
        } else {
            f32x4 xv = *reinterpret_cast<const f32x4*>(x + m * C + c);
            if (MODE == RN_AFFINE_IN) {
                const f32x4 sc = *reinterpret_cast<const f32x4*>(in_scale + b * C + c);
                const f32x4 sh = *reinterpret_cast<const f32x4*>(in_shift + b * C + c);
                xv = xv * sc + sh;
            }
            v[i] = xv;
        }
    }
    float sum = 0.f;
#pragma unroll
    for (int i = 0; i < NV; ++i) sum += (v[i].x + v[i].y) + (v[i].z + v[i].w);
    const float mean = wave_sum(sum) * (1.f / C);
    float sq = 0.f;
#pragma unroll
    for (int i = 0; i < NV; ++i) {
        const f32x4 d = v[i] - mean;
        sq += (d.x * d.x + d.y * d.y) + (d.z * d.z + d.w * d.w);
    }
    const float rstd = 1.f / sqrtf(wave_sum(sq) * (1.f / C) + eps);
#pragma unroll
    for (int i = 0; i < NV; ++i) {
        const int c = (i * 64 + lane) * 4;
        const f32x4 os = *reinterpret_cast<const f32x4*>(out_scale + c);
        const f32x4 oh = *reinterpret_cast<const f32x4*>(out_shift + c);
        const f32x4 o = ((v[i] - mean) * rstd) * os + oh;
        if (s32) store_s32_4(y + m * C, c, o, amax);
        else *reinterpret_cast<f32x4*>(y + m * C + c) = o;
    }
    range_report(status, amax);
}

template <int NV, int R>
__global__ __launch_bounds__(256) void dwconv_ln_kernel(const float* __restrict__ x, float* __restrict__ y, int B, int L,
                                                        const float* __restrict__ dw_w, const float* __restrict__ dw_b,
                                                        const float* __restrict__ out_scale,
                                                        const float* __restrict__ out_shift, float eps, int s32, unsigned* status) {
    constexpr int C = NV * 256;
    const int lane = threadIdx.x & 63;
    float amax = 0.f;
    const int per_clip = (L + R - 1) / R;
    const long wq = (long)blockIdx.x * 4 + (threadIdx.x >> 6);
    if (wq >= (long)B * per_clip) return;
    const int b = (int)(wq / per_clip);
    const int t0 = (int)(wq - (long)b * per_clip) * R;
    const float* xb = x + (long)b * L * C;
    f32x4 v[R][NV];
#pragma unroll
    for (int i = 0; i < NV; ++i) {
        const int c = (i * 64 + lane) * 4;
// ... 635 lines not shown
```

wavtokenizer_amd/csrc/plan.cpp:

```cpp
#include "model.h"

namespace wt {

static bool site_fp32(const wt_plan* P, int site) { return (P->fp32_sites >> site) & 1u; }
static bool plan_fp32(const wt_plan* P) {
    if ((P->flags & WT_PLAN_FLAG_FP32_GEMM) || !P->model->s32_ok) return true;
    if (P->kind == WT_PLAN_SEANET_DECODER) return !P->model->sd_s32_ok || site_fp32(P, SITE_SEADEC);
    if (P->kind == WT_PLAN_ENCODE || P->kind == WT_PLAN_UNIT_LSTM) return site_fp32(P, SITE_ENC);
    if (P->kind == WT_PLAN_HEAD) return site_fp32(P, SITE_HEAD);
    return false;
}
static bool plan_unfused(const wt_plan* P) { return P->flags & WT_PLAN_FLAG_UNFUSED; }
static bool plan_s32(const wt_plan* P) { return !plan_unfused(P) && !plan_fp32(P); }

static int gemm_auto(const wt_plan* P, const GemmArgs& a, int pro, int epi, hipStream_t s) {
    if (P->model->f32_stale.load()) if (int rc = ensure_f32_weights(P->model)) return rc;
    return launch_gemm(a, pro, epi, s);
}

static void set_s32(GemmArgs& a, const S32Copy& c) {
    a.W_hi = c.p; a.acc_scale = c.acc_scale; a.tap_pair = c.tap_pair ? 1 : 0;
}

static int gemm_s32(const GemmArgs& a, int epi, int out, hipStream_t s, const int* mix = nullptr) {
// ... 317 lines not shown
    const wt_arch& ar = M->arch;
    const int B = P->B, L = (int)P->L, D = ar.dim;
    const long Mrows = (long)B * L;
    const int Kb = M->Kb, hop = ar.hop_length;
    const int spec = P->buf("head.spec", (size_t)Mrows * 2 * Kb, s32 ? BUF_S32 : BUF_F32);
    GemmArgs ah = linear_args(M->head_W, M->head_b, Mrows, 2 * Kb, D);
    P->step({xo, spec}, [=](const RunCtx& c) {
        GemmArgs a = ah; a.A = P->ptr(c, xo); a.C = P->ptr(c, spec); a.c_rstride = 2 * Kb; a.head_kb = Kb;
        return dense(P, s32, a, PRO_NONE, EPI_HEAD, OUT_S32, c.stream);
    }, 1, "head.out");
    const int Kq = M->Kq;
    const int parts = P->buf("head.parts", (size_t)4 * Mrows * Kq);
    P->step({spec, parts}, [=](const RunCtx& c) {
        GemmArgs a = linear_args(M->istft_W, nullptr, Mrows, Kq, Kq);
        a.A = P->ptr(c, spec); a.a_rstride = 2 * Kb; a.zA = Kq;
        a.zW = (long)Kq * Kq; a.nz = 4;
        a.C = P->ptr(c, parts); a.c_rstride = Kq; a.zC = (long)Mrows * Kq;
        return dense(P, s32, a, PRO_NONE, EPI_BIAS, OUT_F32, c.stream);
    }, 1, "head.istft");
    P->step({parts}, [=](const RunCtx& c) {
        return launch_istft_ola(P->ptr(c, parts), M->win, M->wsq, c.out_f, B, L, ar.n_fft, hop, Kq, ar.padding_same ? 0 : 1, c.stream);
    }, 1, "head.ola");
}

int build_decode(wt_plan* P) {
    const wt_model* M = P->model;
    const wt_arch& ar = M->arch;
    const int B = P->B, L = (int)P->L, D = ar.dim, I = ar.intermediate_dim, Cin = ar.input_channels;
    const long Mrows = (long)B * L;
    const int Lp = ((L + 31) / 32) * 32;
    const bool s32_plan = plan_s32(P) && (Cin % 32 == 0) && (D % 32 == 0) && (I % 32 == 0);
    auto s32_at = [&](int site) { return s32_plan && !site_fp32(P, site); };
    P->cur_site = SITE_BB_EMBED;
    const bool s32_e = s32_at(SITE_BB_EMBED);
    const int x0 = P->buf("bb.in", (size_t)Mrows * Cin, s32_e ? BUF_S32 : BUF_F32);
    P->step({x0}, [=](const RunCtx& c) { return launch_transpose(c.in_f, P->ptr(c, x0), B, Cin, L, c.stream, s32_e); });
    const int x = P->buf("bb.x", (size_t)Mrows * D);
    GemmArgs ae = zconv_args(M->bb_embed, B, L);
    P->step({x0, x}, [=](const RunCtx& c) {
        GemmArgs a = ae; a.A = P->ptr(c, x0); a.C = P->ptr(c, x);
        return dense(P, s32_e, a, PRO_NONE, EPI_BIAS, OUT_F32, c.stream);
    });
    const bool keep = P->flags & WT_PLAN_FLAG_KEEP_STAGES;
    auto snapshot = [&](const std::string& name) {
        if (!keep) return;
        const int s = P->buf(name, (size_t)Mrows * D);
        P->step({x, s}, [=](const RunCtx& c) {
            WT_HIP_CHECK(hipMemcpyAsync(P->ptr(c, s), P->ptr(c, x), (size_t)Mrows * D * sizeof(float), hipMemcpyDeviceToDevice, c.stream));
            return 0;
        });
    };
    snapshot("bb.embed");
    const int sc = P->buf("bb.gn_scale", (size_t)B * D), sh = P->buf("bb.gn_shift", (size_t)B * D);
    const int gp = P->buf("bb.gn_part", gn_part_floats(B, L, 32));
    const int h1 = P->buf("bb.h1", (size_t)Mrows * D, s32_plan ? BUF_S32 : BUF_F32);
    const int h2 = P->buf("bb.h2", (size_t)Mrows * D);

    auto resnet = [&](const PosRes& r, const std::string& name, int site) {
        P->cur_site = site;
        const bool s32 = s32_at(site);
        P->bufs[h1].fmt = s32 ? BUF_S32 : BUF_F32;
        P->step({x, sc, sh, h1, gp}, [=](const RunCtx& c) {
            return launch_gn_apply(P->ptr(c, x), r.n1w, r.n1b, P->ptr(c, sc), P->ptr(c, sh), P->ptr(c, h1), 1, B, L, D, 32, 1e-6f, c.stream, s32, P->ptr(c, gp));
        }, 1, "res.gn1");
        GemmArgs a1 = zconv_args(r.c1, B, L);
        P->step({h1, h2}, [=](const RunCtx& c) {
            GemmArgs a = a1; a.A = P->ptr(c, h1); a.C = P->ptr(c, h2);
            return dense(P, s32, a, PRO_NONE, EPI_BIAS, OUT_F32, c.stream);
        }, 1, "res.conv1");
        P->step({h2, sc, sh, h1, gp}, [=](const RunCtx& c) {
            return launch_gn_apply(P->ptr(c, h2), r.n2w, r.n2b, P->ptr(c, sc), P->ptr(c, sh), P->ptr(c, h1), 1, B, L, D, 32, 1e-6f, c.stream, s32, P->ptr(c, gp));
        }, 1, "res.gn2");
        GemmArgs a2 = zconv_args(r.c2, B, L);
        P->step({h1, x}, [=](const RunCtx& c) {
            GemmArgs a = a2; a.A = P->ptr(c, h1); a.C = P->ptr(c, x); a.R = P->ptr(c, x); a.r_rstride = D;
            return dense(P, s32, a, PRO_NONE, EPI_BIAS_RES, OUT_F32, c.stream);
        }, 1, "res.conv2");
        snapshot(name);
    };
    resnet(M->res[0], "bb.pos_net.0", SITE_RES0);
    resnet(M->res[1], "bb.pos_net.1", SITE_RES1);
    {
        P->cur_site = SITE_ATTN;
        const bool s32 = s32_at(SITE_ATTN) && M->at_Wqk.s32.p && M->at_Wv.s32.p && M->at_Wp.s32.p;
        const int fmt = s32 ? BUF_S32 : BUF_F32;
        P->bufs[h1].fmt = fmt;
        const int qk = P->buf("bb.attn.qk", (size_t)Mrows * 2 * D, fmt);
        const int vt = P->buf("bb.attn.vt", (size_t)B * D * Lp, fmt);
        const int S = P->buf("bb.attn.s", (size_t)Mrows * Lp);
        const int Ps = s32 ? P->buf("bb.attn.p", (size_t)Mrows * Lp, BUF_S32) : S;
        const int o = P->buf("bb.attn.o", (size_t)Mrows * D, fmt);
        P->step({x, sc, sh, gp, h1}, [=](const RunCtx& c) {
            return launch_gn_apply(P->ptr(c, x), M->at_nw, M->at_nb, P->ptr(c, sc), P->ptr(c, sh), P->ptr(c, h1), 0, B, L, D, 32, 1e-6f, c.stream, s32, P->ptr(c, gp));
        }, 1, "attn.gn");
        GemmArgs aqk = linear_args(M->at_Wqk, M->at_bqk, Mrows, 2 * D, D);
        P->step({h1, qk}, [=](const RunCtx& c) {
            GemmArgs a = aqk; a.A = P->ptr(c, h1); a.C = P->ptr(c, qk);
            return dense(P, s32, a, PRO_NONE, EPI_BIAS, OUT_S32, c.stream);
        }, 1, "attn.qk");
        P->step({h1, vt}, [=](const RunCtx& c) {
            if (int rc = launch_fill_u32(P->ptr(c, vt), 0u, (size_t)B * D * Lp * sizeof(float), c.stream)) return rc;
            GemmArgs a = linear_args(nullptr, M->at_bv, D, L, D);
            a.A = s32 ? static_cast<const float*>(M->at_Wv.s32.p) : M->at_Wv.w; a.acc_scale = M->at_Wv.s32.acc_scale; a.zA = 0;
            a.zW = (long)L * D; a.nz = B;
            a.C = P->ptr(c, vt); a.c_rstride = Lp; a.zC = (long)D * Lp;
            return dense_act(P, s32, a, P->ptr(c, h1), EPI_BIAS_ROW, OUT_S32, c.stream);
        }, 2, "attn.vt");
        P->step({qk, S}, [=](const RunCtx& c) {
            GemmArgs a = linear_args(nullptr, nullptr, L, L, D);
            a.A = P->ptr(c, qk); a.a_rstride = 2 * D; a.zA = (long)L * 2 * D;
            a.w_rstride = 2 * D; a.zW = (long)L * 2 * D; a.nz = B;
            a.C = P->ptr(c, S); a.c_rstride = Lp; a.zC = (long)L * Lp;
            a.alpha = (float)std::pow((double)D, -0.5);
            return dense_act(P, s32, a, P->ptr(c, qk) + D, EPI_SCALE, OUT_F32, c.stream);
        }, 1, "attn.s");
        P->step({S, Ps}, [=](const RunCtx& c) { return launch_softmax(P->ptr(c, S), (int)Mrows, L, Lp, c.stream, s32 ? P->ptr(c, Ps) : nullptr); });
        P->step({Ps, vt, o}, [=](const RunCtx& c) {
            GemmArgs a = linear_args(nullptr, nullptr, L, D, Lp);
            a.A = P->ptr(c, Ps); a.zA = (long)L * Lp;
            a.zW = (long)D * Lp; a.nz = B;
            a.C = P->ptr(c, o); a.c_rstride = D; a.zC = (long)L * D;
            return dense_act(P, s32, a, P->ptr(c, vt), EPI_BIAS, OUT_S32, c.stream);
        }, 1, "attn.o");
        GemmArgs ap = linear_args(M->at_Wp, M->at_bp, Mrows, D, D);
        P->step({o, x}, [=](const RunCtx& c) {
            GemmArgs a = ap; a.A = P->ptr(c, o); a.C = P->ptr(c, x); a.R = P->ptr(c, x); a.r_rstride = D;
            return dense(P, s32, a, PRO_NONE, EPI_BIAS_RES, OUT_F32, c.stream);
        }, 1, "attn.proj");
        snapshot("bb.pos_net.2");
    }
    resnet(M->res[2], "bb.pos_net.3", SITE_RES2);
    resnet(M->res[3], "bb.pos_net.4", SITE_RES3);
    P->cur_site = SITE_CNX0;
    const int xc = P->buf(keep ? "bb.x2" : "bb.norm", (size_t)Mrows * D);
    P->step({x, gp, sc, sh}, [=](const RunCtx& c) {
        return launch_gn_stats(P->ptr(c, x), M->gn5w, M->gn5b, P->ptr(c, sc), P->ptr(c, sh), B, L, D, 32, 1e-6f, c.stream, P->ptr(c, gp));
    });
    P->step({x, sc, sh, xc}, [=](const RunCtx& c) {
        return launch_rownorm(RN_AFFINE_IN, P->ptr(c, x), P->ptr(c, xc), B, L, D, nullptr, nullptr, P->ptr(c, sc),
                              P->ptr(c, sh), M->ada_s + (size_t)c.bw_id * D, M->ada_h + (size_t)c.bw_id * D, 1e-6f, c.stream);
    });
    if (keep) {
        const int sn = P->buf("bb.norm", (size_t)Mrows * D);
        P->step({xc, sn}, [=](const RunCtx& c) {
            WT_HIP_CHECK(hipMemcpyAsync(P->ptr(c, sn), P->ptr(c, xc), (size_t)Mrows * D * sizeof(float), hipMemcpyDeviceToDevice, c.stream));
            return 0;
        });
    }
    const int nrm = P->buf("bb.cnx.norm", (size_t)Mrows * D, s32_plan ? BUF_S32 : BUF_F32);
    const int mid = P->buf("bb.cnx.mid", (size_t)Mrows * I, s32_plan ? BUF_S32 : BUF_F32);
    for (int i = 0; i < ar.num_layers; ++i) {
        const CnxBlock cb = M->cnx[i];
        P->cur_site = SITE_CNX0 + i;
        const bool s32 = s32_at(SITE_CNX0 + i);
        P->bufs[nrm].fmt = P->bufs[mid].fmt = s32 ? BUF_S32 : BUF_F32;
        P->step({xc, nrm}, [=](const RunCtx& c) {
            return launch_rownorm(RN_DWCONV, P->ptr(c, xc), P->ptr(c, nrm), B, L, D, cb.dw_w, cb.dw_b, nullptr, nullptr,
                                  cb.ada_s + (size_t)c.bw_id * D, cb.ada_h + (size_t)c.bw_id * D, 1e-6f, c.stream, s32);
        });
        GemmArgs a1 = linear_args(cb.W1, cb.b1, Mrows, I, D);
        P->step({nrm, mid}, [=](const RunCtx& c) {
            GemmArgs a = a1; a.A = P->ptr(c, nrm); a.C = P->ptr(c, mid);
            return dense(P, s32, a, PRO_NONE, EPI_BIAS_GELU, OUT_S32, c.stream);
        }, 1, "cnx.pwconv1");
        GemmArgs a2 = linear_args(cb.W2, cb.b2, Mrows, D, I);
        P->step({mid, xc}, [=](const RunCtx& c) {
            GemmArgs a = a2; a.A = P->ptr(c, mid); a.C = P->ptr(c, xc); a.R = P->ptr(c, xc); a.r_rstride = D; a.gamma = cb.gamma;
            return dense(P, s32, a, PRO_NONE, EPI_BIAS_GAMMA_RES, OUT_F32, c.stream);
        }, 1, "cnx.pwconv2");
        if (keep && (i == 0 || i == ar.num_layers / 2 - 1 || i == ar.num_layers - 1)) {
            const int s = P->buf("bb.convnext." + std::to_string(i), (size_t)Mrows * D);
            P->step({xc, s}, [=](const RunCtx& c) {
                WT_HIP_CHECK(hipMemcpyAsync(P->ptr(c, s), P->ptr(c, xc), (size_t)Mrows * D * sizeof(float), hipMemcpyDeviceToDevice, c.stream));
                return 0;
            });
        }
    }
    P->cur_site = SITE_HEAD;
    const bool s32 = s32_at(SITE_HEAD);
    const int xo = P->buf("bb.out", (size_t)Mrows * D, s32 ? BUF_S32 : BUF_F32);
    P->step({xc, xo}, [=](const RunCtx& c) {
        if (int rc = launch_rownorm(RN_PLAIN, P->ptr(c, xc), P->ptr(c, xo), B, L, D, nullptr, nullptr, nullptr, nullptr,
                                    M->fln_w, M->fln_b, 1e-6f, c.stream, s32)) return rc;
        if (c.aux && s32)
            return launch_rownorm(RN_PLAIN, P->ptr(c, xc), c.aux, B, L, D, nullptr, nullptr, nullptr, nullptr, M->fln_w,
                                  M->fln_b, 1e-6f, c.stream, 0);
        if (c.aux) WT_HIP_CHECK(hipMemcpyAsync(c.aux, P->ptr(c, xo), (size_t)Mrows * D * sizeof(float), hipMemcpyDeviceToDevice, c.stream));
        return 0;
    });
    plan_head(P, xo, s32);
    return 0;
}

int build_head(wt_plan* P) {
    const wt_model* M = P->model;
    const int B = P->B, L = (int)P->L, D = M->arch.dim;
    const long Mrows = (long)B * L;
    P->cur_site = SITE_HEAD;
    const bool s32 = plan_s32(P) && (D % 32 == 0) && M->head_W.s32.p && M->istft_W.s32.p;
    const int xo = P->buf("head.in", (size_t)Mrows * D, s32 ? BUF_S32 : BUF_F32);
    P->step({xo}, [=](const RunCtx& c) {
        if (s32) return launch_split_s32(c.in_f, P->ptr(c, xo), Mrows * D, c.stream);
        WT_HIP_CHECK(hipMemcpyAsync(P->ptr(c, xo), c.in_f, (size_t)Mrows * D * sizeof(float), hipMemcpyDeviceToDevice, c.stream));
        return 0;
    });
    plan_head(P, xo, s32);
    return 0;
// ... 131 lines not shown
```

wavtokenizer_amd/csrc/weights.cpp:

```cpp
#include "model.h"

namespace wt {

static int upload(wt_model* M, const std::vector<float>& h, float** out) {
    void* d = nullptr;
    size_t bytes = std::max<size_t>(h.size(), 4) * sizeof(float);
    WT_HIP_CHECK(hipMalloc(&d, bytes));
    M->allocs.push_back(d);
    M->alloc_bytes.push_back(bytes);
    WT_HIP_CHECK(hipMemcpy(d, h.data(), h.size() * sizeof(float), hipMemcpyHostToDevice));
    M->weight_bytes += (int64_t)h.size() * sizeof(float);
    *out = static_cast<float*>(d);
    return 0;
}
static int upload_raw(wt_model* M, const float* src, int64_t n, float** out) {
    std::vector<float> h(src, src + n);
    return upload(M, h, out);
}

static std::vector<float> fold_wn(const float* g, const float* v, int d0, int64_t inner) {
    std::vector<float> w((size_t)d0 * inner);
    for (int o = 0; o < d0; ++o) {
        double ss = 0.0;
        for (int64_t i = 0; i < inner; ++i) { double x = v[o * inner + i]; ss += x * x; }
// ... 60 lines not shown
        const size_t blk = prow / 16, li = prow % 16;
        const int S = k / 16, e = (k % 16) / 4, lk = k % 4;
        dst[blk * 16 * Ktot + (size_t)S * 256 + (size_t)(lk * 16 + li) * 4 + e] = v;
    };
    std::vector<_Float16> W0h((size_t)4 * H * H * 2), W1h((size_t)4 * H * 2 * H * 2);
    auto put16 = [&](std::vector<_Float16>& dst, size_t prow, int Ktot, int k, float v) {
        const size_t blk = prow / 16, li = prow % 16;
        const int P = k / 32, r = k % 32, pp = (r / 16) * 4 + (r % 16) / 4, lk = r % 4;
        const size_t base = blk * 16 * Ktot * 2 + (size_t)P * 1024 + (size_t)(lk * 16 + li) * 8 + pp;
        const _Float16 h = (_Float16)v;
        dst[base] = h;
        dst[base + 512] = (_Float16)((v - (float)h) * 2048.f);
    };
    std::vector<_Float16> Wp(H == 512 ? (size_t)3 * 2048 * 512 * 2 : 0);
    auto putp = [&](int role, size_t prow, int k, float v) {
        if (Wp.empty()) return;
        const size_t wg = prow / 64, tile = (prow % 64) / 16, li = prow % 16;
        const int blk = k / 32, lk = (k % 32) / 8, pp = k % 8;
        const size_t base = ((((size_t)role * 32 + wg) * 4 + tile) * 16 + blk) * 2 * 64 * 8 + (size_t)(lk * 16 + li) * 8 + pp;
        const _Float16 h = (_Float16)v;
        Wp[base] = h;
        Wp[base + 64 * 8] = (_Float16)((v - (float)h) * 2048.f);
    };
    for (const float* wsrc : {whh0, wih1, whh1})
        for (size_t i = 0; i < (size_t)4 * H * H; ++i)
            if (!(std::fabs(wsrc[i]) < 65504.f)) *split_ok = false;
    for (int g = 0; g < 4; ++g)
        for (int j = 0; j < H; ++j) {
            const size_t src = (size_t)g * H + j;
            const size_t dst = (size_t)(j / 4) * 16 + g * 4 + (j % 4);
            std::memcpy(&Wih0[dst * H], &wih0[src * H], H * sizeof(float));
            for (int k = 0; k < H; ++k) {
                put(W0, dst, H, k, whh0[src * H + k]);
                put(W1, dst, 2 * H, k, wih1[src * H + k]);
                put(W1, dst, 2 * H, H + k, whh1[src * H + k]);
                put16(W0h, dst, H, k, whh0[src * H + k]);
                put16(W1h, dst, 2 * H, k, wih1[src * H + k]);
                put16(W1h, dst, 2 * H, H + k, whh1[src * H + k]);
                putp(0, dst, k, whh0[src * H + k]);
                putp(1, dst, k, wih1[src * H + k]);
                putp(2, dst, k, whh1[src * H + k]);
            }
            b0[dst] = bih0[src] + bhh0[src];
            b1[dst] = bih1[src] + bhh1[src];
        }
    if (int rc = upload_gemm(M, Wih0, 4 * H, H, &out->Wih0)) return rc;
    if (int rc = upload(M, b0, &out->b0)) return rc;
    if (int rc = upload(M, W0, &out->W0)) return rc;
    if (int rc = upload(M, W1, &out->W1)) return rc;
    {
        std::vector<float> t0(W0.size()), t1(W1.size());
        std::memcpy(t0.data(), W0h.data(), t0.size() * sizeof(float));
        std::memcpy(t1.data(), W1h.data(), t1.size() * sizeof(float));
        if (int rc = upload(M, t0, &out->W0h)) return rc;
        if (int rc = upload(M, t1, &out->W1h)) return rc;
        if (!Wp.empty()) {
            std::vector<float> tp(Wp.size() / 2);
            std::memcpy(tp.data(), Wp.data(), tp.size() * sizeof(float));
            if (int rc = upload(M, tp, &out->Wp)) return rc;
        }
    }
    return upload(M, b1, &out->b1);
}

static int build_cat(wt_model* M, const ConvW& sc, const ConvW& c1, ConvW* cat) {
    if (sc.k != 1 || c1.k != 1 || sc.cout != c1.cout) return 0;
    const int C = sc.cout, K1 = sc.cin, K2 = c1.cin;
    std::vector<float> ws((size_t)C * K1), w1((size_t)C * K2), bs(C), b1(C), w((size_t)C * (K1 + K2)), b(C);
    WT_HIP_CHECK(hipMemcpy(ws.data(), sc.w, ws.size() * sizeof(float), hipMemcpyDeviceToHost));
    WT_HIP_CHECK(hipMemcpy(w1.data(), c1.w, w1.size() * sizeof(float), hipMemcpyDeviceToHost));
    WT_HIP_CHECK(hipMemcpy(bs.data(), sc.b, bs.size() * sizeof(float), hipMemcpyDeviceToHost));
    WT_HIP_CHECK(hipMemcpy(b1.data(), c1.b, b1.size() * sizeof(float), hipMemcpyDeviceToHost));
    for (int n = 0; n < C; ++n) {
        std::memcpy(&w[(size_t)n * (K1 + K2)], &ws[(size_t)n * K1], K1 * sizeof(float));
        std::memcpy(&w[(size_t)n * (K1 + K2) + K1], &w1[(size_t)n * K2], K2 * sizeof(float));
        b[n] = bs[n] + b1[n];
    }
    if (int rc = upload(M, w, &cat->w)) return rc;
    if (int rc = upload(M, b, &cat->b)) return rc;
    cat->cout = C; cat->cin = K1 + K2; cat->k = 1;
    return 0;
}

static const char* ENC = "feature_extractor.encodec.encoder.model.";
static const char* DEC = "feature_extractor.encodec.decoder.model.";
static const char* VQK = "feature_extractor.encodec.quantizer.vq.layers.0._codebook.";

int build_model(wt_model* M, TensorMap& tm) {
    const wt_arch& a = M->arch;
    const int nf = 32, H = 512;
    M->H = H;
    {
        const float* g = tm.get(std::string(ENC) + "0.conv.conv.weight_g", nf);
        const float* v = tm.get(std::string(ENC) + "0.conv.conv.weight_v", (int64_t)nf * 7);
        const float* b = tm.get(std::string(ENC) + "0.conv.conv.bias", nf);
        if (!g || !v || !b) return WT_ERR_MISSING_TENSOR;
        std::vector<float> w = fold_wn(g, v, nf, 7);
        std::vector<float> p((size_t)7 * nf);
        for (int c = 0; c < nf; ++c)
            for (int j = 0; j < 7; ++j) p[(size_t)j * nf + c] = w[(size_t)c * 7 + j];
        if (int rc = upload(M, p, &M->e0_w)) return rc;
        if (int rc = upload_raw(M, b, nf, &M->e0_b)) return rc;
    }
    int idx = 1, mult = 1;
    for (int r : M->enc_ratios) {
        ResStage st;
        st.C = mult * nf; st.r = r;
        const std::string p = std::string(ENC) + std::to_string(idx);
        if (int rc = load_wn_conv(M, tm, p + ".block.1.conv.conv", st.C / 2, st.C, 3, &st.c3)) return rc;
        if (int rc = load_wn_conv(M, tm, p + ".block.3.conv.conv", st.C, st.C / 2, 1, &st.c1)) return rc;
        if (int rc = load_wn_conv(M, tm, p + ".shortcut.conv.conv", st.C, st.C, 1, &st.sc)) return rc;
        if (int rc = load_wn_conv(M, tm, std::string(ENC) + std::to_string(idx + 2) + ".conv.conv", 2 * st.C, st.C, 2 * r, &st.down)) return rc;
        if (!resblock_fusable(st.C)) if (int rc = build_cat(M, st.sc, st.c1, &st.cat)) return rc;
        M->stages.push_back(st);
        idx += 3; mult *= 2;
    }
    if (mult * nf != H) { set_error("encoder width after the last ratio must be 512"); return WT_ERR_INVALID; }
    if (int rc = load_lstm(M, tm, std::string(ENC) + std::to_string(idx), H, &M->enc_lstm, &M->s32_ok)) return rc;
    if (int rc = load_wn_conv(M, tm, std::string(ENC) + std::to_string(idx + 2) + ".conv.conv", 512, H, 7, &M->enc_final)) return rc;

    {
        const float* inited = tm.get(std::string(VQK) + "inited", 1);
        const float* e = tm.get(std::string(VQK) + "embed", (int64_t)a.vq_bins * 512);
        if (!inited || !e) return WT_ERR_MISSING_TENSOR;
        if (inited[0] != 1.0f) {
            set_error("codebook buffer `inited` is not 1: the reference would run k-means on the first forward (core_vq.py:140-151)");
            return WT_ERR_NOT_INITED;
        }
        std::vector<float> all((size_t)a.num_quantizers * a.vq_bins * 512);
        std::memcpy(all.data(), e, (size_t)a.vq_bins * 512 * sizeof(float));
        for (int q = 1; q < a.num_quantizers; ++q) {
            const std::string pq = "feature_extractor.encodec.quantizer.vq.layers." + std::to_string(q) + "._codebook.";
            const float* eq = tm.get(pq + "embed", (int64_t)a.vq_bins * 512);
            if (!eq) return WT_ERR_MISSING_TENSOR;
            std::memcpy(all.data() + (size_t)q * a.vq_bins * 512, eq, (size_t)a.vq_bins * 512 * sizeof(float));
        }
        M->embed.rows = a.vq_bins; M->embed.cols = 512;
        if (int rc = upload(M, all, &M->embed.w)) return rc;
        std::vector<float> ee(a.vq_bins);
        for (int n = 0; n < a.vq_bins; ++n) {
            float s = 0.f;
            for (int c = 0; c < 512; ++c) s += e[(size_t)n * 512 + c] * e[(size_t)n * 512 + c];
            ee[n] = s;
        }
        if (int rc = upload(M, ee, &M->ee)) return rc;
    }

    const int D = a.dim, I = a.intermediate_dim, A = a.adanorm_num_embeddings;
    if (int rc = load_plain_conv(M, tm, "backbone.embed", D, a.input_channels, 7, &M->bb_embed)) return rc;
    const int ridx[4] = {0, 1, 3, 4};
    for (int i = 0; i < 4; ++i) {
        const std::string p = "backbone.pos_net." + std::to_string(ridx[i]);
        PosRes& r = M->res[i];
        if (int rc = load_vec(M, tm, p + ".norm1.weight", D, &r.n1w)) return rc;
        if (int rc = load_vec(M, tm, p + ".norm1.bias", D, &r.n1b)) return rc;
        if (int rc = load_vec(M, tm, p + ".norm2.weight", D, &r.n2w)) return rc;
        if (int rc = load_vec(M, tm, p + ".norm2.bias", D, &r.n2b)) return rc;
        if (int rc = load_plain_conv(M, tm, p + ".conv1", D, D, 3, &r.c1)) return rc;
        if (int rc = load_plain_conv(M, tm, p + ".conv2", D, D, 3, &r.c2)) return rc;
    }
    {
        const std::string p = "backbone.pos_net.2";
        if (int rc = load_vec(M, tm, p + ".norm.weight", D, &M->at_nw)) return rc;
        if (int rc = load_vec(M, tm, p + ".norm.bias", D, &M->at_nb)) return rc;
        const float* wq = tm.get(p + ".q.weight", (int64_t)D * D);
        const float* wk = tm.get(p + ".k.weight", (int64_t)D * D);
        const float* bq = tm.get(p + ".q.bias", D);
        const float* bk = tm.get(p + ".k.bias", D);
        if (!wq || !wk || !bq || !bk) return WT_ERR_MISSING_TENSOR;
        std::vector<float> wqk((size_t)2 * D * D), bqk(2 * D);
        std::memcpy(&wqk[0], wq, (size_t)D * D * sizeof(float));
        std::memcpy(&wqk[(size_t)D * D], wk, (size_t)D * D * sizeof(float));
        std::memcpy(&bqk[0], bq, D * sizeof(float));
        std::memcpy(&bqk[D], bk, D * sizeof(float));
        if (int rc = upload_gemm(M, wqk, 2 * D, D, &M->at_Wqk)) return rc;
        if (int rc = upload(M, bqk, &M->at_bqk)) return rc;
        if (int rc = load_gemm(M, tm, p + ".v.weight", D, D, &M->at_Wv)) return rc;
        if (int rc = load_vec(M, tm, p + ".v.bias", D, &M->at_bv)) return rc;
        if (int rc = load_gemm(M, tm, p + ".proj_out.weight", D, D, &M->at_Wp)) return rc;
        if (int rc = load_vec(M, tm, p + ".proj_out.bias", D, &M->at_bp)) return rc;
    }
    if (int rc = load_vec(M, tm, "backbone.pos_net.5.weight", D, &M->gn5w)) return rc;
    if (int rc = load_vec(M, tm, "backbone.pos_net.5.bias", D, &M->gn5b)) return rc;
    if (A <= 0) { set_error("only the AdaLayerNorm (adanorm_num_embeddings > 0) backbone is implemented"); return WT_ERR_INVALID; }
    if (int rc = load_vec(M, tm, "backbone.norm.scale.weight", (int64_t)A * D, &M->ada_s)) return rc;
    if (int rc = load_vec(M, tm, "backbone.norm.shift.weight", (int64_t)A * D, &M->ada_h)) return rc;
    for (int i = 0; i < a.num_layers; ++i) {
        const std::string p = "backbone.convnext." + std::to_string(i);
        CnxBlock c;
        const float* dw = tm.get(p + ".dwconv.weight", (int64_t)D * 7);
        if (!dw) return WT_ERR_MISSING_TENSOR;
        std::vector<float> dwp((size_t)7 * D);
        for (int ch = 0; ch < D; ++ch)
            for (int j = 0; j < 7; ++j) dwp[(size_t)j * D + ch] = dw[(size_t)ch * 7 + j];
        if (int rc = upload(M, dwp, &c.dw_w)) return rc;
        if (int rc = load_vec(M, tm, p + ".dwconv.bias", D, &c.dw_b)) return rc;
        if (int rc = load_vec(M, tm, p + ".norm.scale.weight", (int64_t)A * D, &c.ada_s)) return rc;
        if (int rc = load_vec(M, tm, p + ".norm.shift.weight", (int64_t)A * D, &c.ada_h)) return rc;
        if (int rc = load_gemm(M, tm, p + ".pwconv1.weight", I, D, &c.W1)) return rc;
        if (int rc = load_vec(M, tm, p + ".pwconv1.bias", I, &c.b1)) return rc;
        if (int rc = load_gemm(M, tm, p + ".pwconv2.weight", D, I, &c.W2)) return rc;
        if (int rc = load_vec(M, tm, p + ".pwconv2.bias", D, &c.b2)) return rc;
        if (int rc = load_vec(M, tm, p + ".gamma", D, &c.gamma)) return rc;
        M->cnx.push_back(c);
    }
    if (int rc = load_vec(M, tm, "backbone.final_layer_norm.weight", D, &M->fln_w)) return rc;
    if (int rc = load_vec(M, tm, "backbone.final_layer_norm.bias", D, &M->fln_b)) return rc;

    {
        const int N = a.n_fft, hop = a.hop_length;
        if (N % hop != 0 || N % 2 != 0 || (N - hop) % 2 != 0) {
            set_error("ISTFT kernel needs n_fft to be an even multiple of hop_length"); return WT_ERR_INVALID;
        }
        if (N % 4 != 0) { set_error("ISTFT kernel needs n_fft % 4 == 0"); return WT_ERR_INVALID; }
        const int bins = N / 2 + 1;
        const int Q = N / 4;
        const int Kq = ((Q + 1 + 31) / 32) * 32;
        const int Kb = 2 * Kq;
        const int R = N / hop;
        M->Kb = Kb; M->Kq = Kq; M->bins_f = bins; M->R = R;
        const float* w = tm.get("head.out.weight", (int64_t)(N + 2) * D);
        const float* b = tm.get("head.out.bias", N + 2);
        const float* win = tm.get("head.istft.window", N);
        if (!w || !b || !win) return WT_ERR_MISSING_TENSOR;
        auto slot_bin = [&](int s) { int f = s < Kq ? 2 * s : 2 * (s - Kq) + 1; return f <= N / 2 && (s < Kq || s - Kq < Q) ? f : -1; };
        std::vector<float> wp((size_t)2 * Kb * D, 0.f), bp((size_t)2 * Kb, 0.f);
        for (int sl = 0; sl < Kb; ++sl) {
            const int f = slot_bin(sl);
            if (f < 0) continue;
            const size_t pm = (size_t)(sl / 16) * 32 + (sl % 16), pp = pm + 16;
            std::memcpy(&wp[pm * D], &w[(size_t)f * D], D * sizeof(float));
            std::memcpy(&wp[pp * D], &w[(size_t)(bins + f) * D], D * sizeof(float));
            bp[pm] = b[f];
            bp[pp] = b[bins + f];
        }
        if (int rc = upload_gemm(M, wp, 2 * Kb, D, &M->head_W)) return rc;
        if (int rc = upload(M, bp, &M->head_b)) return rc;
        std::vector<float> basis((size_t)4 * Kq * Kq, 0.f);
        const double two_pi = 6.283185307179586476925286766559;
        for (int n = 0; n <= Q; ++n)
            for (int g = 0; g <= Q; ++g) {
                const int fe = 2 * g, fo = 2 * g + 1;
                const bool edge = (fe == 0) || (fe == N / 2);
                const double ce = (edge ? 1.0 : 2.0) / (double)N, co = 2.0 / (double)N;
                const double the = two_pi * (double)(((long)fe * n) % N) / (double)N;
                const double tho = two_pi * (double)(((long)fo * n) % N) / (double)N;
                basis[((size_t)0 * Kq + n) * Kq + g] = (float)(ce * std::cos(the));
                basis[((size_t)2 * Kq + n) * Kq + g] = edge ? 0.f : (float)(ce * std::sin(the));
                if (g < Q) {
                    basis[((size_t)1 * Kq + n) * Kq + g] = (float)(co * std::cos(tho));
                    basis[((size_t)3 * Kq + n) * Kq + g] = (float)(co * std::sin(tho));
                }
            }
        if (int rc = upload_gemm(M, basis, 4 * Kq, Kq, &M->istft_W)) return rc;
        if (int rc = upload_raw(M, win, N, &M->win)) return rc;
        std::vector<float> wsq(N);
        for (int n = 0; n < N; ++n) wsq[n] = win[n] * win[n];
        if (int rc = upload(M, wsq, &M->wsq)) return rc;
    }

    M->has_seadec = tm.has(std::string(DEC) + "0.conv.conv.weight_v");
    if (M->has_seadec) {
        int m2 = 1 << a.n_ratios;
// ... 50 lines not shown
    }
    return 0;
}

float s32_weight_scale(float amax) {
    if (!(amax > 0.f) || (amax >= 0x1p-6f && amax < 0x1p12f)) return 1.f;
    int e = 0;
    (void)std::frexp(amax, &e);
    return std::ldexp(1.f, 1 - e);
}
static int add_s32(wt_model* M, const float* w, long n, S32Copy* out, bool* split_ok = nullptr, bool gemm_only = false) {
    if (!w || n <= 0 || (n % 32)) return 0;
    if (!split_ok) split_ok = &M->s32_ok;
    std::vector<float> h((size_t)n);
    WT_HIP_CHECK(hipMemcpy(h.data(), w, (size_t)n * sizeof(float), hipMemcpyDeviceToHost));
    float amax = 0.f;
    bool finite = true;
    for (long i = 0; i < n; ++i) {
        const float v = std::fabs(h[i]);
        if (!(v <= 3.0e38f)) finite = false;
        else amax = std::max(amax, v);
    }
    if (!finite) *split_ok = false;
    M->w_amax = std::max(M->w_amax, amax);
    const float scale = finite ? s32_weight_scale(amax) : 1.f;
    float* scale_dev = nullptr;
    if (scale != 1.f) {
        if (int rc = upload(M, std::vector<float>{scale}, &scale_dev)) return rc;
        out->acc_scale = 1.f / scale;
    }
    void* d = nullptr;
    WT_HIP_CHECK(hipMalloc(&d, (size_t)n * 4));
    M->allocs.push_back(d);
    M->alloc_bytes.push_back((size_t)n * 4);
    M->weight_bytes += n * 4;
    if (int rc = launch_split_s32(w, d, n, nullptr, scale_dev)) return rc;
    out->p = d;
    if (gemm_only && finite) M->lazy_f32.push_back({w, d, (int64_t)n, scale});
    return 0;
}

int build_splits(wt_model* M) {
    auto conv32 = [&](ConvW& c, bool gemm_only = true) { return (c.cin % 32) ? 0 : add_s32(M, c.w, (long)c.cout * c.k * c.cin, &c.s32, nullptr, gemm_only); };
    auto gemm32 = [&](GemmW& g, bool* split_ok = nullptr, bool gemm_only = true) { return add_s32(M, g.w, (long)g.rows * g.cols, &g.s32, split_ok, gemm_only); };
    auto conv32sd = [&](ConvW& c) { return (c.cin % 32) ? 0 : add_s32(M, c.w, (long)c.cout * c.k * c.cin, &c.s32, &M->sd_s32_ok, true); };
    for (ResStage& st : M->stages) {
        if (st.down.cin % 32 == 0 && st.down.k == 2 * st.r && st.down.k <= 32) {
            const long n = (long)st.down.cout * st.down.k * st.down.cin;
            std::vector<float> h((size_t)n), pk((size_t)n);
            WT_HIP_CHECK(hipMemcpy(h.data(), st.down.w, (size_t)n * sizeof(float), hipMemcpyDeviceToHost));
            for (int co = 0; co < st.down.cout; ++co)
                for (int q = 0; q < st.down.k; ++q) {
                    const int tap = (q >> 1) + (q & 1) * st.r;
                    std::memcpy(&pk[((size_t)co * st.down.k + q) * st.down.cin], &h[((size_t)co * st.down.k + tap) * st.down.cin],
                                st.down.cin * sizeof(float));
                }
            float* dpk = nullptr;
            if (int rc = upload(M, pk, &dpk)) return rc;
            if (int rc = add_s32(M, dpk, n, &st.down.s32)) return rc;
            M->lazy_f32.push_back({dpk, nullptr, (int64_t)n, 1.f});
            st.down.s32.tap_pair = true;
        } else
        if (int rc = conv32(st.down, false)) return rc;
        const bool fused = resblock_fusable(st.C);
        if (int rc = conv32(st.c3, !fused)) return rc;
        if (int rc = conv32(st.c1, !fused)) return rc;
        if (int rc = conv32(st.sc, !fused)) return rc;
        if (st.cat.w) if (int rc = conv32(st.cat)) return rc;
    }
    if (int rc = gemm32(M->enc_lstm.Wih0)) return rc;
    if (int rc = conv32(M->enc_final)) return rc;
    if (int rc = gemm32(M->embed, nullptr, false)) return rc;
    if (int rc = conv32(M->bb_embed)) return rc;
    for (int i = 0; i < 4; ++i) {
        if (int rc = conv32(M->res[i].c1)) return rc;
        if (int rc = conv32(M->res[i].c2)) return rc;
    }
    for (CnxBlock& c : M->cnx) {
        if (int rc = gemm32(c.W1)) return rc;
        if (int rc = gemm32(c.W2)) return rc;
    }
    if (int rc = gemm32(M->head_W)) return rc;
    if (int rc = gemm32(M->istft_W)) return rc;
    if (int rc = gemm32(M->at_Wqk)) return rc;
    if (int rc = gemm32(M->at_Wv)) return rc;
    if (int rc = gemm32(M->at_Wp)) return rc;
    if (M->has_seadec) {
        if (int rc = conv32sd(M->sd_first)) return rc;
        if (int rc = gemm32(M->sd_lstm.Wih0, &M->sd_s32_ok)) return rc;
        for (SeaDecStage& st : M->sd_stages) {
            if (st.tr_wp.w && st.cin % 16 == 0) if (int rc = gemm32(st.tr_wp, &M->sd_s32_ok)) return rc;
            if (resblock_fusable(st.cout)) continue;
            if (int rc = conv32sd(st.sc)) return rc;
            if (int rc = conv32sd(st.c3)) return rc;
            if (int rc = conv32sd(st.c1)) return rc;
            if (st.cat.w) if (int rc = conv32sd(st.cat)) return rc;
        }
    }
    WT_HIP_CHECK(hipDeviceSynchronize());
    return 0;
}


static constexpr uint32_t PACK_MAGIC = 0x4b505457u;
static constexpr int32_t PACK_VERSION = 7;

static uint64_t arch_hash_of(const wt_arch& a) {
    uint64_t h = 1469598103934665603ull;
    auto mix = [&](const void* p, size_t n) { for (size_t i = 0; i < n; ++i) { h ^= static_cast<const unsigned char*>(p)[i]; h *= 1099511628211ull; } };
    mix(&a, sizeof(a));
    mix(&PACK_VERSION, sizeof(PACK_VERSION));
    return h;
}

struct Archive {
    bool saving;
    std::vector<char>* out = nullptr;
    const char* in = nullptr;
    size_t pos = 0, n = 0;
    bool ok = true;
    const std::map<const void*, int>* index = nullptr;
    const std::vector<void*>* allocs = nullptr;
    const std::vector<size_t>* alloc_bytes = nullptr;
    void raw(void* p, size_t bytes) {
        if (saving) { const char* c = static_cast<const char*>(p); out->insert(out->end(), c, c + bytes); }
        else { if (!ok || bytes > n - pos) { ok = false; std::memset(p, 0, bytes); return; } std::memcpy(p, in + pos, bytes); pos += bytes; }
    }
    int32_t count(size_t have, int32_t limit) {
        int32_t c = (int32_t)have;
        pod(c);
        if (!saving && (c < 0 || c > limit)) { ok = false; c = 0; }
        return c;
    }
    template <class T> void pod(T& v) { raw(&v, sizeof(T)); }
    template <class T> void ptr(T*& p) {
        int32_t idx = -1;
        int64_t off = 0;
        if (saving && p) {
            auto it = index->upper_bound(static_cast<const void*>(p));
            if (it == index->begin()) { ok = false; }
            else { --it; idx = it->second; off = reinterpret_cast<const char*>(p) - static_cast<const char*>(it->first); }
        }
        pod(idx); pod(off);
        if (!saving) {
            if (idx < 0) p = nullptr;
            else if (!ok || idx >= (int)allocs->size() || off < 0 || (size_t)off >= (*alloc_bytes)[idx]) { ok = false; p = nullptr; }
            else p = reinterpret_cast<T*>(static_cast<char*>((*allocs)[idx]) + off);
        }
    }
    void s32(S32Copy& s) { ptr(s.p); pod(s.acc_scale); pod(s.tap_pair); }
    void conv(ConvW& c) { ptr(c.w); ptr(c.b); pod(c.cout); pod(c.cin); pod(c.k); s32(c.s32); }
    void gemm(GemmW& g) { ptr(g.w); pod(g.rows); pod(g.cols); s32(g.s32); }
    void lstm(LstmW& l) { gemm(l.Wih0); ptr(l.b0); ptr(l.W0); ptr(l.W1); ptr(l.b1); ptr(l.W0h); ptr(l.W1h); ptr(l.Wp); }
};

static void archive_model(Archive& ar, wt_model* M) {
    ar.pod(M->hop); ar.pod(M->H); ar.pod(M->weight_bytes); ar.pod(M->s32_ok); ar.pod(M->sd_s32_ok); ar.pod(M->w_amax);
    int32_t n = ar.count(M->enc_ratios.size(), 8);
    M->enc_ratios.resize(n);
    for (int& r : M->enc_ratios) ar.pod(r);
    ar.ptr(M->e0_w); ar.ptr(M->e0_b); ar.pod(M->e0_k); ar.pod(M->e0_c);
    n = ar.count(M->stages.size(), 8); M->stages.resize(n);
    for (ResStage& st : M->stages) { ar.conv(st.c3); ar.conv(st.c1); ar.conv(st.sc); ar.conv(st.down); ar.conv(st.cat); ar.pod(st.C); ar.pod(st.r); }
    ar.lstm(M->enc_lstm); ar.conv(M->enc_final); ar.gemm(M->embed); ar.ptr(M->ee);
    ar.conv(M->bb_embed);
    for (PosRes& r : M->res) { ar.ptr(r.n1w); ar.ptr(r.n1b); ar.ptr(r.n2w); ar.ptr(r.n2b); ar.conv(r.c1); ar.conv(r.c2); }
    ar.ptr(M->at_nw); ar.ptr(M->at_nb); ar.gemm(M->at_Wqk); ar.ptr(M->at_bqk); ar.gemm(M->at_Wv); ar.ptr(M->at_bv); ar.gemm(M->at_Wp); ar.ptr(M->at_bp);
    ar.ptr(M->gn5w); ar.ptr(M->gn5b); ar.ptr(M->ada_s); ar.ptr(M->ada_h);
    n = ar.count(M->cnx.size(), 64); M->cnx.resize(n);
    for (CnxBlock& c : M->cnx) { ar.ptr(c.dw_w); ar.ptr(c.dw_b); ar.ptr(c.ada_s); ar.ptr(c.ada_h); ar.gemm(c.W1); ar.ptr(c.b1); ar.gemm(c.W2); ar.ptr(c.b2); ar.ptr(c.gamma); }
    ar.ptr(M->fln_w); ar.ptr(M->fln_b); ar.gemm(M->head_W); ar.ptr(M->head_b);
    ar.pod(M->Kb); ar.pod(M->Kq); ar.pod(M->bins_f); ar.pod(M->R);
    ar.gemm(M->istft_W); ar.ptr(M->wsq); ar.ptr(M->win);
    ar.pod(M->has_seadec); ar.conv(M->sd_first); ar.lstm(M->sd_lstm);
    n = ar.count(M->sd_stages.size(), 8); M->sd_stages.resize(n);
    for (SeaDecStage& st : M->sd_stages) {
        ar.ptr(st.tr_w); ar.gemm(st.tr_wp); ar.ptr(st.tr_b); ar.pod(st.cin); ar.pod(st.cout); ar.pod(st.k); ar.pod(st.r);
        ar.conv(st.c3); ar.conv(st.c1); ar.conv(st.sc); ar.conv(st.cat);
    }
    ar.ptr(M->sd_last_w); ar.ptr(M->sd_last_b);
    n = ar.count(M->lazy_f32.size(), 1 << 12); M->lazy_f32.resize(n);
    for (wt_model::LazyF32& z : M->lazy_f32) { ar.ptr(z.w); ar.ptr(z.s32); ar.pod(z.n); ar.pod(z.scale); }
}

struct PackHeader {
    uint32_t magic;
    int32_t version;
    wt_arch arch;
    uint64_t arch_hash;
    uint64_t n_allocs, struct_bytes, payload_bytes;
    uint64_t body_hash;
};

static uint64_t body_hash_of(const char* p, size_t n) {
    uint64_t h[4] = {0x9e3779b97f4a7c15ull, 0xc2b2ae3d27d4eb4full, 0x165667b19e3779f9ull, 0x27d4eb2f165667c5ull};
    const uint64_t K = 0x100000001b3ull * 0x9e3779b1ull | 1ull;
    size_t i = 0;
    for (; i + 32 <= n; i += 32) {
        uint64_t w[4];
        std::memcpy(w, p + i, 32);
        for (int l = 0; l < 4; ++l) { h[l] = (h[l] ^ w[l]) * K; h[l] ^= h[l] >> 29; }
    }
    for (; i < n; ++i) { h[0] = (h[0] ^ (unsigned char)p[i]) * K; h[0] ^= h[0] >> 29; }
    h[0] = (h[0] ^ (uint64_t)n) * K;
    return (h[0] ^ (h[1] * 3) ^ (h[2] * 5) ^ (h[3] * 7)) * K;
}

static constexpr uint64_t PACK_NOT_STORED = 1ull << 63;

static std::vector<bool> lazy_allocs(const wt_model* M) {
    std::vector<bool> lazy(M->allocs.size(), false);
    for (const wt_model::LazyF32& z : M->lazy_f32)
        for (size_t i = 0; i < M->allocs.size(); ++i)
            if (M->allocs[i] == static_cast<const void*>(z.w)) lazy[i] = true;
    return lazy;
}

size_t model_export_bytes(const wt_model* M) {
    size_t total = sizeof(PackHeader) + M->allocs.size() * sizeof(uint64_t) + (1u << 17);
    const std::vector<bool> lazy = lazy_allocs(M);
    for (size_t i = 0; i < M->allocs.size(); ++i) if (!lazy[i]) total += (M->alloc_bytes[i] + 255) / 256 * 256;
    return total + 256;
}

int model_export(const wt_model* Mc, void* buf, size_t n) {
    wt_model* M = const_cast<wt_model*>(Mc);
    std::map<const void*, int> index;
    for (size_t i = 0; i < M->allocs.size(); ++i) index[M->allocs[i]] = (int)i;
    std::vector<char> st;
    Archive ar;
    ar.saving = true; ar.out = &st; ar.index = &index;
    archive_model(ar, M);
    if (!ar.ok) { set_error("wt_model_export: a model pointer lies outside the model's allocations"); return WT_ERR_INVALID; }
    PackHeader h{};
    h.magic = PACK_MAGIC; h.version = PACK_VERSION; h.arch = M->arch; h.arch_hash = arch_hash_of(M->arch);
    h.n_allocs = M->allocs.size(); h.struct_bytes = st.size();
    if (M->f32_stale.load()) if (int rc = ensure_f32_weights(M)) return rc;
    const std::vector<bool> lazy = lazy_allocs(M);
    size_t pos = sizeof(PackHeader) + M->allocs.size() * sizeof(uint64_t) + st.size();
    pos = (pos + 255) / 256 * 256;
    const size_t payload0 = pos;
    for (size_t i = 0; i < M->allocs.size(); ++i) if (!lazy[i]) pos += (M->alloc_bytes[i] + 255) / 256 * 256;
    h.payload_bytes = pos - payload0;
    if (pos > n) { set_error("wt_model_export: buffer too small (wt_model_export_bytes)"); return WT_ERR_INVALID; }
    char* o = static_cast<char*>(buf);
    std::memset(o, 0, payload0);
    for (size_t i = 0; i < M->allocs.size(); ++i) { uint64_t b = M->alloc_bytes[i] | (lazy[i] ? PACK_NOT_STORED : 0); std::memcpy(o + sizeof(h) + i * 8, &b, 8); }
    std::memcpy(o + sizeof(h) + M->allocs.size() * 8, st.data(), st.size());
    pos = payload0;
    WT_HIP_CHECK(hipDeviceSynchronize());
// ... 27 lines not shown
    if (head_pad > n || h.payload_bytes > n - head_pad) { set_error("packed image: truncated (payload)"); return WT_ERR_INVALID; }
    return WT_OK;
}

size_t packed_bytes(const void* buf, size_t n) {
    if (packed_info(buf, n, nullptr, nullptr, nullptr)) return 0;
    PackHeader h;
    std::memcpy(&h, buf, sizeof(h));
    return (sizeof(PackHeader) + h.n_allocs * 8 + h.struct_bytes + 255) / 256 * 256 + h.payload_bytes;
}

int packed_verify(const void* buf, size_t n) {
    if (int rc = packed_info(buf, n, nullptr, nullptr, nullptr)) return rc;
    PackHeader h;
    std::memcpy(&h, buf, sizeof(h));
    const char* in = static_cast<const char*>(buf);
    const size_t head_pad = (sizeof(PackHeader) + h.n_allocs * 8 + h.struct_bytes + 255) / 256 * 256;
    size_t pos = head_pad;
    for (size_t i = 0; i < h.n_allocs; ++i) {
        uint64_t b;
        std::memcpy(&b, in + sizeof(h) + i * 8, 8);
        if (b & PACK_NOT_STORED) {
            if ((b & ~PACK_NOT_STORED) == 0 || (b & ~PACK_NOT_STORED) > (1ull << 32)) { set_error("packed image: bad size of an unstored array"); return WT_ERR_INVALID; }
            continue;
        }
        if (b == 0 || b > n - pos || (b + 255) / 256 * 256 > n - pos) { set_error("packed image: allocation table does not fit the payload"); return WT_ERR_INVALID; }
        pos += (b + 255) / 256 * 256;
    }
    if (pos - head_pad != h.payload_bytes) { set_error("packed image: allocation table and payload size disagree"); return WT_ERR_INVALID; }
    if (body_hash_of(in + sizeof(h), pos - sizeof(h)) != h.body_hash) { set_error("packed image: content hash mismatch (corrupt file)"); return WT_ERR_INVALID; }
    return WT_OK;
}

static int validate_imported(const wt_model* M) {
    const wt_arch& a = M->arch;
    auto fits = [&](const void* p, size_t bytes) {
        if (!p) return false;
        const char* c = static_cast<const char*>(p);
        for (size_t i = 0; i < M->allocs.size(); ++i) {
            const char* base = static_cast<const char*>(M->allocs[i]);
            if (c >= base && c < base + M->alloc_bytes[i]) return bytes <= (size_t)(base + M->alloc_bytes[i] - c);
        }
        return false;
    };
    auto bad = [](const char* what) { set_error(std::string("packed image: ") + what + " does not match the architecture in its header"); return WT_ERR_INVALID; };
    auto copy_ok = [&](const S32Copy& s, size_t bytes, bool pair_ok) {
        return (!s.p || fits(s.p, bytes)) && s.acc_scale > 0.f && std::isfinite(s.acc_scale) && (pair_ok || !s.tap_pair);
    };
    auto conv_ok = [&](const ConvW& c, int cout, int cin, int k, bool pair_ok = false) {
        const size_t bytes = (size_t)cout * cin * k * 4;
        return c.cout == cout && c.cin == cin && c.k == k && fits(c.w, bytes) && fits(c.b, (size_t)cout * 4) && copy_ok(c.s32, bytes, pair_ok);
    };
    auto gemm_ok = [&](const GemmW& g, int rows, int cols) {
        const size_t bytes = (size_t)rows * cols * 4;
        return g.rows == rows && g.cols == cols && fits(g.w, bytes) && copy_ok(g.s32, bytes, false);
    };
    auto lstm_ok = [&](const LstmW& l, int H) {
        const size_t hh = (size_t)4 * H * H * 4;
        return gemm_ok(l.Wih0, 4 * H, H) && fits(l.b0, (size_t)16 * H) && fits(l.W0, hh) && fits(l.W1, 2 * hh) && fits(l.b1, (size_t)16 * H) &&
               (!l.W0h || fits(l.W0h, hh)) && (!l.W1h || fits(l.W1h, 2 * hh)) &&
               (!l.Wp || fits(l.Wp, (size_t)3 * 32 * 4 * 16 * 2 * 64 * 16));
    };
    const int nf = 32, H = 512, D = a.dim, I = a.intermediate_dim;
    if (a.n_ratios < 1 || a.n_ratios > 8 || a.num_quantizers < 1 || a.num_quantizers > 32 || a.input_channels != 512 || D % 256 || I % 32 || a.num_layers < 1 || a.num_layers > 32 ||
        a.adanorm_num_embeddings < 1 || a.vq_bins < 1 || a.n_fft < 4 || a.hop_length < 1) return bad("the architecture itself");
    int hop = 1;
    for (int i = 0; i < a.n_ratios; ++i) { if (a.ratios[i] < 1 || a.ratios[i] > 64) return bad("a ratio"); hop *= a.ratios[i]; }
    if (M->hop != hop || M->H != H || (int)M->enc_ratios.size() != a.n_ratios || (int)M->stages.size() != a.n_ratios) return bad("the encoder's shape");
    if (M->e0_k != 7 || M->e0_c != nf || !fits(M->e0_w, 7 * nf * 4) || !fits(M->e0_b, nf * 4)) return bad("the first conv");
    int mult = 1;
    for (int i = 0; i < a.n_ratios; ++i) {
        const ResStage& st = M->stages[i];
        const int r = a.ratios[a.n_ratios - 1 - i], C = mult * nf;
        if (M->enc_ratios[i] != r || st.C != C || st.r != r || !conv_ok(st.c3, C / 2, C, 3) || !conv_ok(st.c1, C, C / 2, 1) || !conv_ok(st.sc, C, C, 1) ||
            !conv_ok(st.down, 2 * C, C, 2 * r, true)) return bad("an encoder stage");
        if ((st.cat.w || st.cat.s32.p) && !conv_ok(st.cat, C, C + C / 2, 1)) return bad("a fused shortcut weight");
        mult *= 2;
    }
    if (mult * nf != H || !lstm_ok(M->enc_lstm, H) || !conv_ok(M->enc_final, 512, H, 7)) return bad("the encoder tail");
    if (!gemm_ok(M->embed, a.vq_bins, 512) || !fits(M->embed.w, (size_t)a.num_quantizers * a.vq_bins * 512 * 4) || !fits(M->ee, (size_t)a.vq_bins * 4)) return bad("the codebook");
    if (!conv_ok(M->bb_embed, D, 512, 7)) return bad("backbone.embed");
    for (const PosRes& r : M->res)
        if (!fits(r.n1w, D * 4) || !fits(r.n1b, D * 4) || !fits(r.n2w, D * 4) || !fits(r.n2b, D * 4) || !conv_ok(r.c1, D, D, 3) || !conv_ok(r.c2, D, D, 3)) return bad("a pos_net block");
    if (!fits(M->at_nw, D * 4) || !fits(M->at_nb, D * 4) || !gemm_ok(M->at_Wqk, 2 * D, D) || !fits(M->at_bqk, 2 * D * 4) || !gemm_ok(M->at_Wv, D, D) ||
        !fits(M->at_bv, D * 4) || !gemm_ok(M->at_Wp, D, D) || !fits(M->at_bp, D * 4)) return bad("the attention block");
    const size_t ada = (size_t)a.adanorm_num_embeddings * D * 4;
    if (!fits(M->gn5w, D * 4) || !fits(M->gn5b, D * 4) || !fits(M->ada_s, ada) || !fits(M->ada_h, ada)) return bad("backbone.norm");
    if ((int)M->cnx.size() != a.num_layers) return bad("the ConvNeXt block count");
    for (const CnxBlock& c : M->cnx)
        if (!fits(c.dw_w, (size_t)7 * D * 4) || !fits(c.dw_b, D * 4) || !fits(c.ada_s, ada) || !fits(c.ada_h, ada) || !gemm_ok(c.W1, I, D) || !fits(c.b1, I * 4) ||
            !gemm_ok(c.W2, D, I) || !fits(c.b2, D * 4) || !fits(c.gamma, D * 4)) return bad("a ConvNeXt block");
    const int N = a.n_fft;
    if (N % 4 || N % a.hop_length) return bad("n_fft / hop_length");
    const int Kq = ((N / 4 + 1 + 31) / 32) * 32, Kb = 2 * Kq;
    if (M->Kq != Kq || M->Kb != Kb || M->bins_f != N / 2 + 1 || M->R != N / a.hop_length) return bad("the ISTFT head's shape");
    if (!fits(M->fln_w, D * 4) || !fits(M->fln_b, D * 4) || !gemm_ok(M->head_W, 2 * Kb, D) || !fits(M->head_b, (size_t)2 * Kb * 4) ||
        !gemm_ok(M->istft_W, 4 * Kq, Kq) || !fits(M->win, (size_t)N * 4) || !fits(M->wsq, (size_t)N * 4)) return bad("the ISTFT head");
    if (M->has_seadec) {
        if ((int)M->sd_stages.size() != a.n_ratios || !conv_ok(M->sd_first, (1 << a.n_ratios) * nf, 512, 7) || !lstm_ok(M->sd_lstm, H)) return bad("the SEANetDecoder");
        int m2 = 1 << a.n_ratios;
        for (int i = 0; i < a.n_ratios; ++i) {
            const SeaDecStage& st = M->sd_stages[i];
            const int r = a.ratios[i], cin = m2 * nf, h = cin / 2;
            if (st.cin != cin || st.cout != h || st.k != 2 * r || st.r != r || !fits(st.tr_w, (size_t)2 * r * cin * h * 4) || ((st.tr_wp.w || st.tr_wp.s32.p) && !gemm_ok(st.tr_wp, r * h, 2 * cin)) ||
                !fits(st.tr_b, h * 4) || !conv_ok(st.c3, h / 2, h, 3) || !conv_ok(st.c1, h, h / 2, 1) || !conv_ok(st.sc, h, h, 1)) return bad("a SEANetDecoder stage");
            if ((st.cat.w || st.cat.s32.p) && !conv_ok(st.cat, h, h + h / 2, 1)) return bad("a SEANetDecoder fused shortcut");
            m2 /= 2;
        }
        if (!fits(M->sd_last_w, 7 * nf * 4) || !fits(M->sd_last_b, 4)) return bad("the SEANetDecoder's last conv");
    }
    return WT_OK;
}

int model_import(wt_model* M, const void* buf, size_t n) {
    PackHeader h;
    if (int rc = packed_verify(buf, n)) return rc;
    std::memcpy(&h, buf, sizeof(h));
    M->arch = h.arch;
    const char* in = static_cast<const char*>(buf);
    size_t pos = (sizeof(PackHeader) + h.n_allocs * 8 + h.struct_bytes + 255) / 256 * 256;
    for (size_t i = 0; i < h.n_allocs; ++i) {
        uint64_t b;
        std::memcpy(&b, in + sizeof(h) + i * 8, 8);
        const bool stored = !(b & PACK_NOT_STORED);
        b &= ~PACK_NOT_STORED;
        const size_t padded = (b + 255) / 256 * 256;
        if (stored && pos + padded > n) { set_error("packed image: truncated payload"); return WT_ERR_INVALID; }
        void* d = nullptr;
        WT_HIP_CHECK(hipMalloc(&d, b));
        M->allocs.push_back(d);
        M->alloc_bytes.push_back(b);
        if (stored) {
            WT_HIP_CHECK(hipMemcpy(d, in + pos, b, hipMemcpyHostToDevice));
            pos += padded;
        } else {
            M->f32_stale.store(true);
        }
    }
    Archive ar;
    ar.saving = false; ar.in = in + sizeof(h) + h.n_allocs * 8; ar.n = h.struct_bytes; ar.allocs = &M->allocs; ar.alloc_bytes = &M->alloc_bytes;
    archive_model(ar, M);
    if (!ar.ok || ar.pos != ar.n) { set_error("packed image: model section does not match this library's layout"); return WT_ERR_INVALID; }
    for (const wt_model::LazyF32& z : M->lazy_f32) {
        size_t iw = M->allocs.size(), is = M->allocs.size();
        for (size_t i = 0; i < M->allocs.size(); ++i) {
            if (M->allocs[i] == static_cast<const void*>(z.w)) iw = i;
            if (z.s32 && M->allocs[i] == z.s32) is = i;
        }
        if (iw == M->allocs.size() || z.n <= 0 || (z.n % 32) || (size_t)z.n * 4 > M->alloc_bytes[iw] ||
            (z.s32 && (is == M->allocs.size() || (size_t)z.n * 4 > M->alloc_bytes[is])) || !(z.scale > 0.f) || !std::isfinite(z.scale)) {
            set_error("packed image: bad entry in the list of unstored fp32 arrays"); return WT_ERR_INVALID;
        }
    }
    return validate_imported(M);
}

int ensure_f32_weights(const wt_model* M) {
    std::lock_guard<std::mutex> lock(M->f32_mu);
    if (!M->f32_stale.load()) return WT_OK;
    for (const wt_model::LazyF32& z : M->lazy_f32) {
        if (!z.s32) continue;
        if (int rc = launch_unsplit_s32(z.s32, const_cast<float*>(z.w), (long)z.n, 1.f / z.scale, nullptr)) return rc;
    }
    WT_HIP_CHECK(hipDeviceSynchronize());
    M->f32_stale.store(false);
    return WT_OK;
}

// ... 2 lines not shown
```

Measured before the change: 37920.

## Fold attention Q/K and V/proj weights offline and emit transposed GroupNorm output

Precomputes G = scale·Wkᵀ·Wq (with a bias vector g) and Wo = Wp·Wv (with a folded bias), both on the host in double precision. Attention then runs one D×D projection per row instead of a fused 2D-wide QK projection, a V projection and an output projection, and uses the normalized input directly as the value operand. The GroupNorm tile kernel gains a transposed, padded output, so h1ᵀ for the P·V product comes straight out of the norm instead of from a separate V GEMM. Folding the weights changes rounding and the packed model format (version bump). The key bias is dropped, which is exact because softmax ignores a per-query constant.

```diff
diff --git a/include/wavtokenizer_amd.h b/include/wavtokenizer_amd.h
--- a/include/wavtokenizer_amd.h
+++ b/include/wavtokenizer_amd.h
@@ -143,6 +143,9 @@
 
 int wt_linear(const float* x, const float* w, const float* bias, float* y, int64_t M, int32_t N, int32_t K,
               int32_t f16x3, void* workspace, void* stream);
+
+int wt_attention_fold(int32_t D, const float* wq, const float* bq, const float* wk, const float* wv, const float* bv,
+                      const float* wp, const float* bp, float* G, float* g, float* Wo, float* bo);
 
 int wt_conv1d_s32(const float* x, const float* w, const float* bias, float* y, int32_t B, int64_t T, int32_t Cin,
                   int32_t Cout, int32_t k, int32_t stride, int32_t zero_same, void* workspace, void* stream);
@@ -194,6 +197,7 @@
     const void *p0, *p1, *p2, *p3, *p4, *p5;
     void *y, *y2, *y3;
     uint32_t* status;
+    void* y4;
 } wt_op_desc;
 typedef struct {
     int32_t kernel;
diff --git a/wavtokenizer_amd/_capi.py b/wavtokenizer_amd/_capi.py
--- a/wavtokenizer_amd/_capi.py
+++ b/wavtokenizer_amd/_capi.py
@@ -16,7 +16,7 @@
     "wt_decode", "wt_seanet_decode", "wt_head", "wt_unit_run", "wt_sconv1d", "wt_linear", "wt_conv1d_s32", "wt_vq_workspace_bytes",
     "wt_vq_nearest", "wt_vq_nearest_f32", "wt_resblock", "wt_resblock_down", "wt_gemm_probe_workspace_bytes", "wt_gemm_probe", "wt_op_probe",
     "wt_resampler_create", "wt_resampler_destroy", "wt_resampler_out_length", "wt_convert_audio", "wt_pcm16",
-    "wt_linear_overlap_add", "wt_encode_mixed", "wt_plan_min_clip_length", "wt_sconv_geometry",
+    "wt_linear_overlap_add", "wt_encode_mixed", "wt_plan_min_clip_length", "wt_sconv_geometry", "wt_attention_fold",
 ]
 
 WT_PLAN_ENCODE, WT_PLAN_DECODE, WT_PLAN_SEANET_DECODER, WT_PLAN_HEAD, WT_PLAN_UNIT_LSTM = 0, 1, 2, 3, 4
@@ -72,7 +72,7 @@
     _fields_ = ([(n, c_int32) for n in ("size", "op", "B", "L", "C", "groups", "mode", "flag", "out_s32", "ld", "k", "stride",
                                         "Cout", "n_fft", "hop", "Kq")]
                 + [("eps", c_float), ("n", c_int64)]
-                + [(n, c_void_p) for n in ("x", "p0", "p1", "p2", "p3", "p4", "p5", "y", "y2", "y3", "status")])
+                + [(n, c_void_p) for n in ("x", "p0", "p1", "p2", "p3", "p4", "p5", "y", "y2", "y3", "status", "y4")])
 
 
 class WtOpForm(ctypes.Structure):
@@ -166,6 +166,7 @@
     lib.wt_vq_nearest_f32.argtypes = [c_void_p, c_void_p, c_int64, c_int32, c_int32, c_void_p, c_void_p, c_void_p]
     lib.wt_resblock.argtypes = [c_void_p] * 11 + [c_int32, c_int64, c_int32, c_int32, c_int32, c_int32, c_void_p]
     lib.wt_resblock_down.argtypes = [c_void_p] * 12 + [c_int32, c_int64, c_int32, c_void_p]
+    lib.wt_attention_fold.argtypes = [c_int32] + [c_void_p] * 11
     lib.wt_gemm_probe_workspace_bytes.argtypes = [POINTER(WtGemmDesc)]
     lib.wt_gemm_probe_workspace_bytes.restype = c_size_t
     lib.wt_gemm_probe.argtypes = [POINTER(WtGemmDesc), POINTER(WtLaunchForm), c_void_p, c_void_p]
diff --git a/wavtokenizer_amd/csrc/capi.cpp b/wavtokenizer_amd/csrc/capi.cpp
--- a/wavtokenizer_amd/csrc/capi.cpp
+++ b/wavtokenizer_amd/csrc/capi.cpp
@@ -653,6 +653,13 @@
     return launch_gemm16s(a, EPI_BIAS, f16x3 == 3 ? 1 : 0, s);
 }
 
+int wt_attention_fold(int32_t D, const float* wq, const float* bq, const float* wk, const float* wv, const float* bv,
+                      const float* wp, const float* bp, float* G, float* g, float* Wo, float* bo) {
+    if (D <= 0 || !wq || !bq || !wk || !wv || !bv || !wp || !bp || !G || !g || !Wo || !bo) { set_error("wt_attention_fold: null argument or D <= 0"); return WT_ERR_INVALID; }
+    fold_attention(D, wq, bq, wk, wv, bv, wp, bp, G, g, Wo, bo);
+    return WT_OK;
+}
+
 int wt_conv1d_s32(const float* x, const float* w, const float* bias, float* y, int32_t B, int64_t T, int32_t Cin,
                   int32_t Cout, int32_t k, int32_t stride, int32_t zero_same, void* workspace, void* stream) {
     if (!x || !w || !y || !workspace) { set_error("wt_conv1d_s32: null argument"); return WT_ERR_INVALID; }
@@ -768,7 +775,7 @@
     if (!d || d->size != (int32_t)sizeof(wt_op_desc)) return bad("descriptor missing or of another size");
     if (d->op < WT_OP_GN_APPLY || d->op > WT_OP_S32_AMAX) return bad("unknown op");
     auto al16 = [](const void* p) { return !(reinterpret_cast<uintptr_t>(p) & 15); };
-    const void* ptrs[] = {d->p0, d->p1, d->p2, d->p3, d->p4, d->p5, d->y, d->y2, d->y3};
+    const void* ptrs[] = {d->p0, d->p1, d->p2, d->p3, d->p4, d->p5, d->y, d->y2, d->y3, d->y4};
     for (const void* p : ptrs) if (!al16(p)) return bad("arrays must be 16-byte aligned");
     if (!d->x || (reinterpret_cast<uintptr_t>(d->x) & (d->op == WT_OP_SOFTMAX ? 3 : 15))) return bad("x missing or misaligned");
     if (reinterpret_cast<uintptr_t>(d->status) & 3) return bad("status misaligned");
@@ -779,6 +786,7 @@
     case WT_OP_GN_APPLY: case WT_OP_GN_STATS:
         if (!d->p0 || !d->p1 || !d->y2 || !d->y3 || (d->op == WT_OP_GN_APPLY && !d->y)) return bad("null argument");
         if (d->groups <= 0 || d->C % d->groups || d->C / d->groups > 256 || d->B > 65535) return bad("GroupNorm needs C % groups == 0, at most 256 channels per group, B <= 65535");
+        if (d->op == WT_OP_GN_APPLY && d->y4 && (d->flag || d->C % 4 || (d->out_s32 && d->C % 32))) return bad("the transposed output needs the plain form (no swish) and C % 4 == 0 (S32: C % 32 == 0)");
         break;
     case WT_OP_ROWNORM:
         if (!d->y || !d->p4 || !d->p5) return bad("null argument");
@@ -835,7 +843,7 @@
     switch (d->op) {
     case WT_OP_GN_APPLY:
         rc = launch_gn_apply(F(d->x), F(d->p0), F(d->p1), W(d->y2), W(d->y3), W(d->y), d->flag ? 1 : 0, d->B, d->L, d->C, d->groups, d->eps, s,
-                             d->out_s32 ? 1 : 0, const_cast<float*>(F(d->p2)));
+                             d->out_s32 ? 1 : 0, const_cast<float*>(F(d->p2)), W(d->y4));
         break;
     case WT_OP_GN_STATS:
         rc = launch_gn_stats(F(d->x), F(d->p0), F(d->p1), W(d->y2), W(d->y3), d->B, d->L, d->C, d->groups, d->eps, s, const_cast<float*>(F(d->p2)));
diff --git a/wavtokenizer_amd/csrc/common.h b/wavtokenizer_amd/csrc/common.h
--- a/wavtokenizer_amd/csrc/common.h
+++ b/wavtokenizer_amd/csrc/common.h
@@ -228,7 +228,8 @@
 int launch_gn_stats(const float* x, const float* gamma, const float* beta, float* scale, float* shift, int B, int L,
                     int C, int groups, float eps, hipStream_t s, float* part = nullptr);
 int launch_gn_apply(const float* x, const float* gamma, const float* beta, float* scale, float* shift, float* y,
-                    int swish, int B, int L, int C, int groups, float eps, hipStream_t s, int out_s32 = 0, float* part = nullptr);
+                    int swish, int B, int L, int C, int groups, float eps, hipStream_t s, int out_s32 = 0, float* part = nullptr,
+                    float* yT = nullptr);
 enum RowNormMode : int { RN_DWCONV = 0, RN_PLAIN = 1, RN_AFFINE_IN = 2 };
 int launch_rownorm(int mode, const float* x, float* y, int B, int L, int C, const float* dw_w ,
                    const float* dw_b, const float* in_scale, const float* in_shift, const float* out_scale,
diff --git a/wavtokenizer_amd/csrc/model.h b/wavtokenizer_amd/csrc/model.h
--- a/wavtokenizer_amd/csrc/model.h
+++ b/wavtokenizer_amd/csrc/model.h
@@ -84,8 +84,8 @@
     float* ee = nullptr;
     wt::ConvW bb_embed;
     wt::PosRes res[4];
-    float *at_nw, *at_nb, *at_bqk, *at_bv, *at_bp;
-    wt::GemmW at_Wqk, at_Wv, at_Wp;
+    float *at_nw, *at_nb, *at_g, *at_bo;
+    wt::GemmW at_G, at_Wo;
     float *gn5w, *gn5b, *ada_s, *ada_h;
     std::vector<wt::CnxBlock> cnx;
     float *fln_w, *fln_b;
@@ -285,6 +285,8 @@
 namespace wt {
 
 int build_model(wt_model* M, TensorMap& tm);
+void fold_attention(int D, const float* wq, const float* bq, const float* wk, const float* wv, const float* bv, const float* wp,
+                    const float* bp, float* G, float* g, float* Wo, float* bo);
 int build_splits(wt_model* M);
 float s32_weight_scale(float amax);
 size_t model_export_bytes(const wt_model* M);
diff --git a/wavtokenizer_amd/csrc/ops.hip b/wavtokenizer_amd/csrc/ops.hip
--- a/wavtokenizer_amd/csrc/ops.hip
+++ b/wavtokenizer_amd/csrc/ops.hip
@@ -282,11 +282,12 @@
     return 0;
 }
 
-template <int SWISH>
+template <int SWISH, int TR>
 __global__ __launch_bounds__(512) void gn_tile_kernel(const float* __restrict__ x, const float* __restrict__ gamma,
                                                       const float* __restrict__ beta, float* __restrict__ scale,
                                                       float* __restrict__ shift, float* __restrict__ y, int L, int C,
-                                                      int cg, int GB, float eps, int s32, unsigned* status) {
+                                                      int cg, int GB, float eps, int s32, unsigned* status,
+                                                      float* __restrict__ yT, int Lp) {
     extern __shared__ __attribute__((aligned(16))) float tile[];
     float amax = 0.f;
     __shared__ float s_sc[128], s_sh[128], s_red[8];
@@ -380,9 +381,67 @@
             }
             if (s32) store_s32_4(yb + (long)t * C, c0 + q * 4, o, amax);
             else *reinterpret_cast<f32x4*>(yb + (long)t * C + c0 + q * 4) = o;
+            if (TR) *reinterpret_cast<f32x4*>(tile + t * W + q * 4) = o;
+        }
+    }
+    if (TR) {
+        __syncthreads();
+        float* tb = yT + ((long)b * C + c0) * Lp;
+        for (int e = threadIdx.x; e < (Lp >> 5) * W * 8; e += NT) {
+            const int lq = e & 7, r = e >> 3, j = r / W, c = r - j * W;
+            const int l = j * 32 + lq * 4;
+            f32x4 v;
+#pragma unroll
+            for (int i = 0; i < 4; ++i) v[i] = l + i < L ? tile[(l + i) * W + c] : 0.f;
+            if (s32) store_s32_4(tb + (long)c * Lp, l, v, amax);
+            else *reinterpret_cast<f32x4*>(tb + (long)c * Lp + l) = v;
         }
     }
     range_report(status, amax);
+}
+
+template <int S32>
+__global__ __launch_bounds__(256) void transpose_pad_kernel(const float* __restrict__ in, float* __restrict__ out, int L,
+                                                            int C, int Lp, unsigned* status) {
+    __shared__ unsigned tile[32][33];
+    float amax = 0.f;
+    const int c0 = blockIdx.x * 32, r0 = blockIdx.y * 32, b = blockIdx.z;
+    const int tx = threadIdx.x & 31, ty = threadIdx.x >> 5;
+    for (int i = ty; i < 32; i += 8) {
+        const int r = r0 + i;
+        unsigned w = 0u;
+        if (r < L && c0 + tx < C) {
+            const float* row = in + ((long)b * L + r) * C;
+            if (S32) {
+                const unsigned short* p = reinterpret_cast<const unsigned short*>(row) + (c0 >> 5) * 64 + tx;
+                w = (unsigned)p[0] | ((unsigned)p[32] << 16);
+            } else w = __float_as_uint(row[c0 + tx]);
+        }
+        tile[i][tx] = w;
+    }
+    __syncthreads();
+    for (int i = ty; i < 32; i += 8) {
+        const int c = c0 + i;
+        if (c >= C) continue;
+        const unsigned w = tile[tx][i];
+        float* row = out + ((long)b * C + c) * Lp;
+        if (S32) {
+            unsigned short* q = reinterpret_cast<unsigned short*>(row) + (r0 >> 5) * 64 + tx;
+            q[0] = (unsigned short)(w & 0xffffu);
+            q[32] = (unsigned short)(w >> 16);
+            amax = amax1(amax, (float)__builtin_bit_cast(_Float16, (unsigned short)(w & 0xffffu)));
+        } else row[r0 + tx] = __uint_as_float(w);
+    }
+    range_report(status, amax);
+}
+static int launch_transpose_pad(const float* in, float* out, int B, int L, int C, int Lp, hipStream_t s, int s32) {
+    if (s32 && (C % 32)) { set_error("transpose_pad: S32 rows need C % 32 == 0"); return -1; }
+    if (B > 65535 || Lp / 32 > 65535) { set_error("transpose_pad: too many tiles for one launch"); return -1; }
+    const dim3 grid((C + 31) / 32, Lp / 32, B);
+    if (s32) hipLaunchKernelGGL(transpose_pad_kernel<1>, grid, dim3(256), 0, s, in, out, L, C, Lp, g_launch.status);
+    else hipLaunchKernelGGL(transpose_pad_kernel<0>, grid, dim3(256), 0, s, in, out, L, C, Lp, g_launch.status);
+    WT_HIP_CHECK(hipGetLastError());
+    return 0;
 }
 
 static constexpr int GN_CH = 128;
@@ -500,8 +559,10 @@
 }
 
 int launch_gn_apply(const float* x, const float* gamma, const float* beta, float* scale, float* shift, float* y,
-                    int swish, int B, int L, int C, int groups, float eps, hipStream_t s, int out_s32, float* part) {
+                    int swish, int B, int L, int C, int groups, float eps, hipStream_t s, int out_s32, float* part, float* yT) {
     if (out_s32 && (C % 32)) { set_error("gn_apply: an S32 output needs C % 32 == 0"); return -1; }
+    if (yT && swish) { set_error("gn_apply: the transposed output goes with the plain (no swish) form"); return -1; }
+    const int Lp = (L + 31) / 32 * 32;
     const int cg = C / groups;
     int GB = 0;
     for (int g = 1; g <= groups; ++g)
@@ -510,20 +571,24 @@
         const size_t smem = (size_t)L * GB * cg * sizeof(float);
         static PerDeviceOnce attr_once;
         if (int rc = attr_once.run([&]() -> int {
-            WT_HIP_CHECK(hipFuncSetAttribute(reinterpret_cast<const void*>(gn_tile_kernel<0>), hipFuncAttributeMaxDynamicSharedMemorySize, 96 * 1024));
-            WT_HIP_CHECK(hipFuncSetAttribute(reinterpret_cast<const void*>(gn_tile_kernel<1>), hipFuncAttributeMaxDynamicSharedMemorySize, 96 * 1024));
+            WT_HIP_CHECK(hipFuncSetAttribute(reinterpret_cast<const void*>(gn_tile_kernel<0, 0>), hipFuncAttributeMaxDynamicSharedMemorySize, 96 * 1024));
+            WT_HIP_CHECK(hipFuncSetAttribute(reinterpret_cast<const void*>(gn_tile_kernel<1, 0>), hipFuncAttributeMaxDynamicSharedMemorySize, 96 * 1024));
+            WT_HIP_CHECK(hipFuncSetAttribute(reinterpret_cast<const void*>(gn_tile_kernel<0, 1>), hipFuncAttributeMaxDynamicSharedMemorySize, 96 * 1024));
         return 0;
     })) return rc;
         dim3 grid(groups / GB, B);
         const int nt = GB == 4 ? 512 : 256;
         note_form(OPK_GN_TILE, swish ? 1 : 0, (nt >> 6) == 2 * GB ? 2 : 1, grid, nt, smem);
-        if (swish) hipLaunchKernelGGL(gn_tile_kernel<1>, grid, dim3(nt), smem, s, x, gamma, beta, scale, shift, y, L, C, cg, GB, eps, out_s32, g_launch.status);
-        else hipLaunchKernelGGL(gn_tile_kernel<0>, grid, dim3(nt), smem, s, x, gamma, beta, scale, shift, y, L, C, cg, GB, eps, out_s32, g_launch.status);
+        if (swish) hipLaunchKernelGGL((gn_tile_kernel<1, 0>), grid, dim3(nt), smem, s, x, gamma, beta, scale, shift, y, L, C, cg, GB, eps, out_s32, g_launch.status, (float*)nullptr, 0);
+        else if (yT) hipLaunchKernelGGL((gn_tile_kernel<0, 1>), grid, dim3(nt), smem, s, x, gamma, beta, scale, shift, y, L, C, cg, GB, eps, out_s32, g_launch.status, yT, Lp);
+        else hipLaunchKernelGGL((gn_tile_kernel<0, 0>), grid, dim3(nt), smem, s, x, gamma, beta, scale, shift, y, L, C, cg, GB, eps, out_s32, g_launch.status, (float*)nullptr, 0);
         WT_HIP_CHECK(hipGetLastError());
         return 0;
     }
-    if (part && GB && (cg % 4 == 0) && (C % 4 == 0) && GB * cg <= 128 && GB <= 8)
-        return launch_gn_chunked(x, gamma, beta, scale, shift, y, swish ? 2 : 1, B, L, C, groups, GB, eps, s, out_s32, part);
+    if (part && GB && (cg % 4 == 0) && (C % 4 == 0) && GB * cg <= 128 && GB <= 8) {
+        if (int rc = launch_gn_chunked(x, gamma, beta, scale, shift, y, swish ? 2 : 1, B, L, C, groups, GB, eps, s, out_s32, part)) return rc;
+        return yT ? launch_transpose_pad(y, yT, B, L, C, Lp, s, out_s32) : 0;
+    }
     note_form(OPK_GN_STATS, swish ? 2 : 1, 0, dim3(groups, B), 256);
     if (swish)
         hipLaunchKernelGGL(gn_stats_kernel<2>, dim3(groups, B), dim3(256), 0, s, x, gamma, beta, scale, shift, y, L, C,
@@ -532,7 +597,7 @@
         hipLaunchKernelGGL(gn_stats_kernel<1>, dim3(groups, B), dim3(256), 0, s, x, gamma, beta, scale, shift, y, L, C,
                            C / groups, eps, out_s32, g_launch.status);
     WT_HIP_CHECK(hipGetLastError());
-    return 0;
+    return yT ? launch_transpose_pad(y, yT, B, L, C, Lp, s, out_s32) : 0;
 }
 
 template <int NV, int MODE>
diff --git a/wavtokenizer_amd/csrc/plan.cpp b/wavtokenizer_amd/csrc/plan.cpp
--- a/wavtokenizer_amd/csrc/plan.cpp
+++ b/wavtokenizer_amd/csrc/plan.cpp
@@ -423,47 +423,40 @@
     resnet(M->res[1], "bb.pos_net.1", SITE_RES1);
     {
         P->cur_site = SITE_ATTN;
-        const bool s32 = s32_at(SITE_ATTN) && M->at_Wqk.s32.p && M->at_Wv.s32.p && M->at_Wp.s32.p;
+        const bool s32 = s32_at(SITE_ATTN) && M->at_G.s32.p && M->at_Wo.s32.p;
         const int fmt = s32 ? BUF_S32 : BUF_F32;
         P->bufs[h1].fmt = fmt;
-        const int qk = P->buf("bb.attn.qk", (size_t)Mrows * 2 * D, fmt);
-        const int vt = P->buf("bb.attn.vt", (size_t)B * D * Lp, fmt);
+        const int ht = P->buf("bb.attn.ht", (size_t)B * D * Lp, fmt);
+        const int yq = P->buf("bb.attn.qk", (size_t)Mrows * D, fmt);
         const int S = P->buf("bb.attn.s", (size_t)Mrows * Lp);
         const int Ps = s32 ? P->buf("bb.attn.p", (size_t)Mrows * Lp, BUF_S32) : S;
         const int o = P->buf("bb.attn.o", (size_t)Mrows * D, fmt);
-        P->step({x, sc, sh, gp, h1}, [=](const RunCtx& c) {
-            return launch_gn_apply(P->ptr(c, x), M->at_nw, M->at_nb, P->ptr(c, sc), P->ptr(c, sh), P->ptr(c, h1), 0, B, L, D, 32, 1e-6f, c.stream, s32, P->ptr(c, gp));
+        P->step({x, sc, sh, gp, ht, h1}, [=](const RunCtx& c) {
+            return launch_gn_apply(P->ptr(c, x), M->at_nw, M->at_nb, P->ptr(c, sc), P->ptr(c, sh), P->ptr(c, h1), 0, B, L, D, 32, 1e-6f, c.stream, s32, P->ptr(c, gp),
+                                   P->ptr(c, ht));
         }, 1, "attn.gn");
-        GemmArgs aqk = linear_args(M->at_Wqk, M->at_bqk, Mrows, 2 * D, D);
-        P->step({h1, qk}, [=](const RunCtx& c) {
-            GemmArgs a = aqk; a.A = P->ptr(c, h1); a.C = P->ptr(c, qk);
+        GemmArgs ay = linear_args(M->at_G, M->at_g, Mrows, D, D);
+        P->step({h1, yq}, [=](const RunCtx& c) {
+            GemmArgs a = ay; a.A = P->ptr(c, h1); a.C = P->ptr(c, yq);
             return dense(P, s32, a, PRO_NONE, EPI_BIAS, OUT_S32, c.stream);
-        }, 1, "attn.qk");
-        P->step({h1, vt}, [=](const RunCtx& c) {
-            if (int rc = launch_fill_u32(P->ptr(c, vt), 0u, (size_t)B * D * Lp * sizeof(float), c.stream)) return rc;
-            GemmArgs a = linear_args(nullptr, M->at_bv, D, L, D);
-            a.A = s32 ? static_cast<const float*>(M->at_Wv.s32.p) : M->at_Wv.w; a.acc_scale = M->at_Wv.s32.acc_scale; a.zA = 0;
+        }, 1, "attn.y");
+        P->step({yq, h1, S}, [=](const RunCtx& c) {
+            GemmArgs a = linear_args(nullptr, nullptr, L, L, D);
+            a.A = P->ptr(c, yq); a.zA = (long)L * D;
             a.zW = (long)L * D; a.nz = B;
-            a.C = P->ptr(c, vt); a.c_rstride = Lp; a.zC = (long)D * Lp;
-            return dense_act(P, s32, a, P->ptr(c, h1), EPI_BIAS_ROW, OUT_S32, c.stream);
-        }, 2, "attn.vt");
-        P->step({qk, S}, [=](const RunCtx& c) {
-            GemmArgs a = linear_args(nullptr, nullptr, L, L, D);
-            a.A = P->ptr(c, qk); a.a_rstride = 2 * D; a.zA = (long)L * 2 * D;
-            a.w_rstride = 2 * D; a.zW = (long)L * 2 * D; a.nz = B;
             a.C = P->ptr(c, S); a.c_rstride = Lp; a.zC = (long)L * Lp;
-            a.alpha = (float)std::pow((double)D, -0.5);
-            return dense_act(P, s32, a, P->ptr(c, qk) + D, EPI_SCALE, OUT_F32, c.stream);
+            a.alpha = 1.f;
+            return dense_act(P, s32, a, P->ptr(c, h1), EPI_SCALE, OUT_F32, c.stream);
         }, 1, "attn.s");
         P->step({S, Ps}, [=](const RunCtx& c) { return launch_softmax(P->ptr(c, S), (int)Mrows, L, Lp, c.stream, s32 ? P->ptr(c, Ps) : nullptr); });
-        P->step({Ps, vt, o}, [=](const RunCtx& c) {
+        P->step({Ps, ht, o}, [=](const RunCtx& c) {
             GemmArgs a = linear_args(nullptr, nullptr, L, D, Lp);
             a.A = P->ptr(c, Ps); a.zA = (long)L * Lp;
             a.zW = (long)D * Lp; a.nz = B;
             a.C = P->ptr(c, o); a.c_rstride = D; a.zC = (long)L * D;
-            return dense_act(P, s32, a, P->ptr(c, vt), EPI_BIAS, OUT_S32, c.stream);
+            return dense_act(P, s32, a, P->ptr(c, ht), EPI_BIAS, OUT_S32, c.stream);
         }, 1, "attn.o");
-        GemmArgs ap = linear_args(M->at_Wp, M->at_bp, Mrows, D, D);
+        GemmArgs ap = linear_args(M->at_Wo, M->at_bo, Mrows, D, D);
         P->step({o, x}, [=](const RunCtx& c) {
             GemmArgs a = ap; a.A = P->ptr(c, o); a.C = P->ptr(c, x); a.R = P->ptr(c, x); a.r_rstride = D;
             return dense(P, s32, a, PRO_NONE, EPI_BIAS_RES, OUT_F32, c.stream);
diff --git a/wavtokenizer_amd/csrc/weights.cpp b/wavtokenizer_amd/csrc/weights.cpp
--- a/wavtokenizer_amd/csrc/weights.cpp
+++ b/wavtokenizer_amd/csrc/weights.cpp
@@ -166,6 +166,35 @@
     return 0;
 }
 
+void fold_attention(int D, const float* wq, const float* bq, const float* wk, const float* wv, const float* bv, const float* wp,
+                    const float* bp, float* G, float* g, float* Wo, float* bo) {
+    auto product = [D](bool a_transposed, const float* A, const float* Bm, const float* v, const float* add, double sc, float* out, float* vec) {
+        std::vector<double> acc((size_t)4 * D);
+        for (int n0 = 0; n0 < D; n0 += 4) {
+            const int nb = std::min(4, D - n0);
+            std::fill(acc.begin(), acc.end(), 0.0);
+            double dv[4] = {0.0, 0.0, 0.0, 0.0};
+            for (int m = 0; m < D; ++m) {
+                double a[4] = {0.0, 0.0, 0.0, 0.0};
+                for (int r = 0; r < nb; ++r) a[r] = a_transposed ? A[(size_t)m * D + n0 + r] : A[(size_t)(n0 + r) * D + m];
+                const float* row = Bm + (size_t)m * D;
+                double *a0 = &acc[0], *a1 = &acc[D], *a2 = &acc[(size_t)2 * D], *a3 = &acc[(size_t)3 * D];
+                for (int k = 0; k < D; ++k) {
+                    const double b = row[k];
+                    a0[k] += a[0] * b; a1[k] += a[1] * b; a2[k] += a[2] * b; a3[k] += a[3] * b;
+                }
+                for (int r = 0; r < nb; ++r) dv[r] += a[r] * (double)v[m];
+            }
+            for (int r = 0; r < nb; ++r) {
+                for (int k = 0; k < D; ++k) out[(size_t)(n0 + r) * D + k] = (float)(sc * acc[(size_t)r * D + k]);
+                vec[n0 + r] = (float)(sc * dv[r] + (add ? (double)add[n0 + r] : 0.0));
+            }
+        }
+    };
+    product(true, wk, wq, bq, nullptr, std::pow((double)D, -0.5), G, g);
+    product(false, wp, wv, bv, bp, 1.0, Wo, bo);
+}
+
 static const char* ENC = "feature_extractor.encodec.encoder.model.";
 static const char* DEC = "feature_extractor.encodec.decoder.model.";
 static const char* VQK = "feature_extractor.encodec.quantizer.vq.layers.0._codebook.";
@@ -249,20 +278,18 @@
         if (int rc = load_vec(M, tm, p + ".norm.bias", D, &M->at_nb)) return rc;
         const float* wq = tm.get(p + ".q.weight", (int64_t)D * D);
         const float* wk = tm.get(p + ".k.weight", (int64_t)D * D);
+        const float* wv = tm.get(p + ".v.weight", (int64_t)D * D);
+        const float* wp = tm.get(p + ".proj_out.weight", (int64_t)D * D);
         const float* bq = tm.get(p + ".q.bias", D);
-        const float* bk = tm.get(p + ".k.bias", D);
-        if (!wq || !wk || !bq || !bk) return WT_ERR_MISSING_TENSOR;
-        std::vector<float> wqk((size_t)2 * D * D), bqk(2 * D);
-        std::memcpy(&wqk[0], wq, (size_t)D * D * sizeof(float));
-        std::memcpy(&wqk[(size_t)D * D], wk, (size_t)D * D * sizeof(float));
-        std::memcpy(&bqk[0], bq, D * sizeof(float));
-        std::memcpy(&bqk[D], bk, D * sizeof(float));
-        if (int rc = upload_gemm(M, wqk, 2 * D, D, &M->at_Wqk)) return rc;
-        if (int rc = upload(M, bqk, &M->at_bqk)) return rc;
-        if (int rc = load_gemm(M, tm, p + ".v.weight", D, D, &M->at_Wv)) return rc;
-        if (int rc = load_vec(M, tm, p + ".v.bias", D, &M->at_bv)) return rc;
-        if (int rc = load_gemm(M, tm, p + ".proj_out.weight", D, D, &M->at_Wp)) return rc;
-        if (int rc = load_vec(M, tm, p + ".proj_out.bias", D, &M->at_bp)) return rc;
+        const float* bv = tm.get(p + ".v.bias", D);
+        const float* bp = tm.get(p + ".proj_out.bias", D);
+        if (!wq || !wk || !wv || !wp || !bq || !bv || !bp || !tm.get(p + ".k.bias", D)) return WT_ERR_MISSING_TENSOR;
+        std::vector<float> G((size_t)D * D), g(D), Wo((size_t)D * D), bo(D);
+        fold_attention(D, wq, bq, wk, wv, bv, wp, bp, G.data(), g.data(), Wo.data(), bo.data());
+        if (int rc = upload_gemm(M, G, D, D, &M->at_G)) return rc;
+        if (int rc = upload(M, g, &M->at_g)) return rc;
+        if (int rc = upload_gemm(M, Wo, D, D, &M->at_Wo)) return rc;
+        if (int rc = upload(M, bo, &M->at_bo)) return rc;
     }
     if (int rc = load_vec(M, tm, "backbone.pos_net.5.weight", D, &M->gn5w)) return rc;
     if (int rc = load_vec(M, tm, "backbone.pos_net.5.bias", D, &M->gn5b)) return rc;
@@ -479,9 +506,8 @@
     }
     if (int rc = gemm32(M->head_W)) return rc;
     if (int rc = gemm32(M->istft_W)) return rc;
-    if (int rc = gemm32(M->at_Wqk)) return rc;
-    if (int rc = gemm32(M->at_Wv)) return rc;
-    if (int rc = gemm32(M->at_Wp)) return rc;
+    if (int rc = gemm32(M->at_G)) return rc;
+    if (int rc = gemm32(M->at_Wo)) return rc;
     if (M->has_seadec) {
         if (int rc = conv32sd(M->sd_first)) return rc;
         if (int rc = gemm32(M->sd_lstm.Wih0, &M->sd_s32_ok)) return rc;
@@ -500,7 +526,7 @@
 
 
 static constexpr uint32_t PACK_MAGIC = 0x4b505457u;
-static constexpr int32_t PACK_VERSION = 7;
+static constexpr int32_t PACK_VERSION = 8;
 
 static uint64_t arch_hash_of(const wt_arch& a) {
     uint64_t h = 1469598103934665603ull;
@@ -562,7 +588,7 @@
     ar.lstm(M->enc_lstm); ar.conv(M->enc_final); ar.gemm(M->embed); ar.ptr(M->ee);
     ar.conv(M->bb_embed);
     for (PosRes& r : M->res) { ar.ptr(r.n1w); ar.ptr(r.n1b); ar.ptr(r.n2w); ar.ptr(r.n2b); ar.conv(r.c1); ar.conv(r.c2); }
-    ar.ptr(M->at_nw); ar.ptr(M->at_nb); ar.gemm(M->at_Wqk); ar.ptr(M->at_bqk); ar.gemm(M->at_Wv); ar.ptr(M->at_bv); ar.gemm(M->at_Wp); ar.ptr(M->at_bp);
+    ar.ptr(M->at_nw); ar.ptr(M->at_nb); ar.gemm(M->at_G); ar.ptr(M->at_g); ar.gemm(M->at_Wo); ar.ptr(M->at_bo);
     ar.ptr(M->gn5w); ar.ptr(M->gn5b); ar.ptr(M->ada_s); ar.ptr(M->ada_h);
     n = ar.count(M->cnx.size(), 64); M->cnx.resize(n);
     for (CnxBlock& c : M->cnx) { ar.ptr(c.dw_w); ar.ptr(c.dw_b); ar.ptr(c.ada_s); ar.ptr(c.ada_h); ar.gemm(c.W1); ar.ptr(c.b1); ar.gemm(c.W2); ar.ptr(c.b2); ar.ptr(c.gamma); }
@@ -756,8 +782,8 @@
     if (!conv_ok(M->bb_embed, D, 512, 7)) return bad("backbone.embed");
     for (const PosRes& r : M->res)
         if (!fits(r.n1w, D * 4) || !fits(r.n1b, D * 4) || !fits(r.n2w, D * 4) || !fits(r.n2b, D * 4) || !conv_ok(r.c1, D, D, 3) || !conv_ok(r.c2, D, D, 3)) return bad("a pos_net block");
-    if (!fits(M->at_nw, D * 4) || !fits(M->at_nb, D * 4) || !gemm_ok(M->at_Wqk, 2 * D, D) || !fits(M->at_bqk, 2 * D * 4) || !gemm_ok(M->at_Wv, D, D) ||
-        !fits(M->at_bv, D * 4) || !gemm_ok(M->at_Wp, D, D) || !fits(M->at_bp, D * 4)) return bad("the attention block");
+    if (!fits(M->at_nw, D * 4) || !fits(M->at_nb, D * 4) || !gemm_ok(M->at_G, D, D) || !fits(M->at_g, D * 4) || !gemm_ok(M->at_Wo, D, D) ||
+        !fits(M->at_bo, D * 4)) return bad("the attention block");
     const size_t ada = (size_t)a.adanorm_num_embeddings * D * 4;
     if (!fits(M->gn5w, D * 4) || !fits(M->gn5b, D * 4) || !fits(M->ada_s, ada) || !fits(M->ada_h, ada)) return bad("backbone.norm");
     if ((int)M->cnx.size() != a.num_layers) return bad("the ConvNeXt block count");
```

After: 38330 (median of 3 runs). No clear change (+1.1%).
